# yao24/MPAS-Model

Hardware: AMD Instinct MI355X
Metric: dycore cell-updates/sec (nCells×nVertLevels/step) at 1/2/4/8 MI355X; % HBM roofline (higher is better)
Workload: dtype f64; 1 GPU; x1.163842 dry dycore, 56 levels, dt=360s (BASELINE.json configs[2] mesh; one full atm_srk3 per step); nCells=163842, nVertLevels=56, num_scalars=1, split_steps=3, acoustic_substeps=2, parallelism=single block, owned_cells_rank0=163842, halo_cells_rank0=0, hip_graph=True

## Files before the change

### mpas-model_amd/csrc/dycore.hip

```cpp
#include <hip/hip_runtime.h>
#include <rccl/rccl.h>

#include <algorithm>
#include <cmath>
#include <cstdio>
#include <cstring>
#include <functional>
#include <map>
#include <set>
#include <string>
#include <tuple>
#include <vector>
#include <unistd.h>

#ifdef MPAS_API_TAG
#include "api_rename.h"
#endif
#include "../../include/mpas_dycore.h"
#include "p2p_wire.h"
#include "kernels.hip"
#include "halo.hip"
#include "summary.hip"
#include "lbc.hip"
#include "model_init.hip"
// ... 67 lines not shown
  XSeg* d_pre = nullptr;
  XSeg* d_post = nullptr;
  int npre = 0, npost = 0, maxn_pre = 0, maxn_post = 0;
  double* sendbuf = nullptr;
  double* recvbuf = nullptr;
  std::vector<XMsg> rsend, rrecv;
  bool warmed = false;
  bool fused_pack = false;
  std::vector<PackMap> pack;
  bool fused_unpack = false;
  std::vector<UnpackMap> unpack;
  int fused_rec = 0;
  std::vector<XPack> rpk_cell, rpk_edge;
  std::vector<XUnpack> rup_cell, rup_edge;
  bool p2p = false;
  int p2p_id = -1;
  unsigned long long* p2p_cnt = nullptr;
  P2PGet* d_get = nullptr;
  int nget = 0, get_chunks = 0;
  unsigned long long** d_ready = nullptr;
  int nready = 0;
  const unsigned long long** d_cons = nullptr;
  int ncons = 0;
  bool pull = false;
  std::vector<XSeg> h_pre, h_post;
  std::vector<const std::vector<int32_t>*> h_pre_idx;
  std::vector<int64_t> h_pre_off, h_post_off;
  XSeg* d_local = nullptr;
  int nlocal = 0, maxn_local = 0;
  P2PSeg* d_pseg = nullptr;
  int2* d_chunk = nullptr;
  int nchunk = 0, npeer_work = 0;
  P2PPeer* d_peer = nullptr;
  bool skip_pull = false;
};

struct XField {
  const char* pool;
  const char* name;
  int tl;
  unsigned layers;
};
constexpr unsigned ALL_LAYERS = 0x7u;

}

struct mpas_dyc_ctx {
  Config cf{};
  int index_qv = 0;
  int device = 0;
  bool host_only = false;
  hipStream_t stream = nullptr;
  std::vector<Block> blk;
  int cur = 0;
  std::string err;
  hipEvent_t ev[8] = {};
  bool use_graph = false;
  bool graph_ran = false;
  std::map<std::string, hipGraphExec_t> graphs;
  std::map<std::string, double> graph_dt;
  int rank = 0, nranks = 1;
  ncclComm_t comm = nullptr;
  bool rccl_local = false;
  int loopback = 0;
  int p2p = 0;
  unsigned long long* p2p_flags = nullptr;
  int* p2p_status = nullptr;
  int* p2p_status_host = nullptr;
  std::vector<unsigned long long*> p2p_peer_flags;
  std::map<std::pair<int, uint64_t>, void*> p2p_fields;
  int p2p_nr = 0;
  int p2p_next = 0;
  std::vector<XField> p2p_open;
  bool p2p_pending = false;
  bool p2p_merge = true;
  bool p2p_pull = true;
  int p2p_release = 1;
  bool u_local = true;
  int halo_trim = 3;
  bool late_issue = false;
  bool overlap_all = false;
  bool fuse_tend_acoustic = true;
  bool fold_substep_avg = true;
  bool fold_rk1_edges = true;
  bool fuse_recover_diag = true;
  std::vector<XField> late_fs;
  bool late_pending = false;
  bool fused_pack_enabled = true;
  bool plain_exchange = false;
  bool lbc = false;
  bool planning = false;
  std::set<std::string> planned;
  std::map<std::string, XPlan> plans;
  std::vector<std::string>* record = nullptr;
  hipStream_t xstream = nullptr;
  hipEvent_t xfork = nullptr, xjoin = nullptr;
  int overlap = -1;
  bool bnd_ready = false;
  int physics = 0;
  int summary_flags = MPAS_DYC_PRINT_GLOBAL_MINMAX_VEL;
  int summary_tl = 0;
  IauState iau;
  ConvDiagState convdiag;
  MicropState microp;
  int64_t graph_captures = 0;
  bool tail_pending = false;
  bool profile = false;
  bool in_async = false;
  std::vector<hipEvent_t> prof_exposed, prof_rccl;
  hipEvent_t prof_step[2] = {};
  double prof_out[5] = {};
  char last_key[256] = {0};
  double* sum_gather = nullptr;
  mpas_dyc_allgather_fn host_allgather = nullptr;
  void* host_user = nullptr;
};

namespace {

#define HIPCHK(x)                                                                     \
  do {                                                                                \
    hipError_t e_ = (x);                                                              \
    if (e_ != hipSuccess) {                                                           \
      ctx->err = std::string(#x) + ": " + hipGetErrorString(e_);                      \
      return MPAS_DYC_EHIP;                                                           \
    }                                                                                 \
  } while (0)

#define NCCLCHK(x)                                                                    \
  do {                                                                                \
    ncclResult_t r_ = (x);                                                            \
    if (r_ != ncclSuccess) {                                                          \
      ctx->err = std::string(#x) + ": " + ncclGetErrorString(r_);                     \
      return MPAS_DYC_ECOMM;                                                          \
    }                                                                                 \
  } while (0)

#define CHK(x)                 \
  do {                         \
    int r__ = (x);             \
    if (r__) return r__;       \
  } while (0)

int64_t nloc(const Block& b, Loc l) {
  switch (l) {
    case L_CELL: return b.d.nCells + 1;
    case L_EDGE: return b.d.nEdges + 1;
    case L_VERTEX: return b.d.nVertices + 1;
    default: return 1;
  }
}

int64_t field_elems(const Block& b, const Field& f) { return nloc(b, f.loc) * f.inner; }
int64_t field_bytes(const Block& b, const Field& f) { return field_elems(b, f) * (f.is_int ? 4 : 8); }

bool is_host_0d(const Field& f) {
  return f.pool == "mesh" && (f.name == "cf1" || f.name == "cf2" || f.name == "cf3");
}

Field& add(Block& c, const char* pool, const char* name, Loc loc, int64_t inner, int ntl = 1, bool is_int = false,
           Target t = T_NONE) {
  Field f;
  f.pool = pool;
  f.name = name;
  f.loc = loc;
  f.inner = inner;
// ... 505 lines not shown
void swap_theta(mpas_dyc_ctx* ctx) {
  for (auto& b : ctx->blk) {
    Field* f = find(b, "state", "theta_m");
    std::swap(f->buf[0], f->buf[1]);
    f->flip ^= 1;
  }
}

Ptrs stage_pre(const Ptrs& p0, bool first_substep) {
  Ptrs p = p0;
  p.ru = p.ru_save;
  p.rw = p.rw_save;
  p.rw_rd = p.rw_save;
  p.rtheta_p = p.rtheta_p_save;
  p.theta_m2 = p.theta_m1;
  p.ru_rd = p.ru_save;
  p.theta_m2_rd = p.theta_m1;
  if (first_substep) {
    p.u2 = p.u1;
    p.w2 = p.w1;
    p.w2_rd = p.w1;
    p.rho_zz2 = p.rho_zz1;
    p.rho_zz2_rd = p.rho_zz1;
  }
  return p;
}

Ptrs stage_fin(const Ptrs& p0, bool first_substep) {
  Ptrs p = p0;
  p.rw_rd = p.rw_save;
  p.ru_rd = p.ru_save;
  p.theta_m2_rd = p.theta_m1;
  if (first_substep) {
    p.w2_rd = p.w1;
    p.rho_zz2_rd = p.rho_zz1;
  }
  return p;
}

int step_rotations(const Config& cf) { return cf.split_dynamics_transport ? cf.dynamics_split_steps : 1; }

void apply_step_rotations(mpas_dyc_ctx* ctx) {
  const int n = step_rotations(ctx->cf);
  if (n & 1) rotate_saves(ctx);
  if ((n - 1) & 1) swap_theta(ctx);
}

std::string layout_sig(mpas_dyc_ctx* ctx) {
  Block& b = ctx->blk[0];
  return std::to_string(ctx->cur) + "." + std::to_string(find(b, "diag", "ru")->rot_pos) + "." +
         std::to_string(find(b, "state", "theta_m")->flip);
}

struct Layout {
  std::vector<std::tuple<Field*, void*, void*, int, int>> f;
};
Layout save_layout(mpas_dyc_ctx* ctx) {
  Layout l;
  for (auto& b : ctx->blk)
    for (auto& f : b.fields)
      if (f.rot >= 0 || (f.pool == "state" && f.name == "theta_m")) l.f.emplace_back(&f, f.buf[0], f.buf[1], f.rot_pos, f.flip);
  return l;
}
void restore_layout(const Layout& l) {
  for (const auto& t : l.f) {
    Field* f = std::get<0>(t);
    f->buf[0] = std::get<1>(t);
    f->buf[1] = std::get<2>(t);
    f->rot_pos = std::get<3>(t);
    f->flip = std::get<4>(t);
  }
}

void rk_integration_setup(mpas_dyc_ctx* ctx, const Dims& d, const Ptrs& p) {
  CopyList c{};
  c.src[0] = p.scalars1;
  c.dst[0] = p.scalars2;
  c.n[0] = (int64_t)(d.nCells + 1) * d.K * d.ns;
  const unsigned gx = (unsigned)std::min<int64_t>((c.n[0] + 255) / 256, 2048);
  if (!ctx->planning) hipLaunchKernelGGL(k_copy_many, dim3(gx, 1), dim3(256), 0, ctx->stream, c);
}


void vert_imp_coefs(mpas_dyc_ctx* ctx, const Dims& d, const Ptrs& p, double dts) {
  if (g_vic == 2) {
    LAUNCH(k_vert_imp_coefs<true>, std::max(d.nCellsSolve, 1), d, p, dts, ctx->cf.epssm);
    if (d.nCellsSolve > 0 && !ctx->planning)
      hipLaunchKernelGGL(k_vert_imp_lu, dim3((unsigned)((d.nCellsSolve + 63) / 64)), dim3(64), 0, ctx->stream, d, p);
  } else if (pair_layout(d) && g_vic == 1) {
    LAUNCH_PE((k_vert_imp_coefs_p<false>), (k_vert_imp_coefs_p<true>), std::max(d.nCellsSolve, 1), d, p, dts, ctx->cf.epssm);
  } else {
    LAUNCH(k_vert_imp_coefs<false>, std::max(d.nCellsSolve, 1), d, p, dts, ctx->cf.epssm);
  }
}

bool fused_recover(const Dims& d) { return batched(d) && (d.maxEdges == 6 || d.maxEdges == 7); }

struct TendAcoustic {
  Ptrs pf;
  bool fin;
  double dts, rdt, invNs;
  int keep_pp, dl, store_tend;
  int sa;
  double sa_inv;
};
bool tend_acoustic_fused(const mpas_dyc_ctx* ctx, int rk_step, int nsub) {
#ifdef MPAS_WIDE
  return false;
#else
  if (!ctx->fuse_tend_acoustic || needs_exchange(ctx) || ctx->lbc || ctx->blk.size() != 1) return false;
  const Dims& d = ctx->blk[0].d;
  return fuse_smlstep(d) && fused_recover(d) && !(rk_step == 1 && nsub > 1);
#endif
}
bool substep_avg_folded(const mpas_dyc_ctx* ctx) {
#ifdef MPAS_WIDE
  return false;
#else
  if (!ctx->fold_substep_avg || needs_exchange(ctx) || ctx->lbc || ctx->blk.size() != 1) return false;
  if (!ctx->cf.split_dynamics_transport) return false;
  const Dims& d = ctx->blk[0].d;
  return pair_layout(d) && fused_recover(d) && d.nCellsSolve == d.nCells && d.nEdgesSolve == d.nEdges &&
         d.n_bnd_edges == 0;
#endif
}
bool rk1_edge_folded(const mpas_dyc_ctx* ctx, const Dims& d) {
#ifdef MPAS_WIDE
  return false;
#else
  return ctx->fold_rk1_edges && pair_layout(d) && !(ctx->cf.v_mom_eddy_visc2 > 0.0);
#endif
}
bool recover_diag_fused(const mpas_dyc_ctx* ctx) {
#ifdef MPAS_WIDE
  return false;
#else
  if (!ctx->fuse_recover_diag || needs_exchange(ctx) || ctx->lbc || ctx->blk.size() != 1) return false;
  if (ctx->cf.scalar_advection && !ctx->cf.split_dynamics_transport) return false;
  return pair_layout(ctx->blk[0].d);
#endif
}
void stage_sub_steps(const Config& cf, int n[3]) {
  const int nss = cf.number_of_sub_steps;
  n[0] = cf.time_integration_order == 3 ? 1 : std::max(1, nss / 2);
  n[1] = std::max(1, nss / 2);
  n[2] = nss;
}

void dyn_tend(mpas_dyc_ctx* ctx, const Dims& d, const Ptrs& p, int rk_step, double dt, int part = 0,
              bool hdiv_done = false, bool last = true, XPack tp = XPack{}, const TendAcoustic* ta = nullptr) {
  const Config& cf = ctx->cf;
  DynTendScal s{};
  s.rk_step = rk_step;
  s.store_phys_diag = last ? 1 : 0;
  s.dt = dt;
  s.invDt = 1.0 / dt;
  s.coef_3rd_order = cf.coef_3rd_order;
  s.c_s = cf.smagorinsky_coef;
  if (cf.horiz_mixing_smag) {
    s.h_mom_eddy_visc4 = cf.visc4_2dsmag * (cf.len_disp * cf.len_disp * cf.len_disp);
    s.h_theta_eddy_visc4 = s.h_mom_eddy_visc4;
  } else {
    s.h_mom_eddy_visc4 = cf.h_mom_eddy_visc4;
    s.h_theta_eddy_visc4 = cf.h_theta_eddy_visc4;
  }
  if (cf.rayleigh_damp_u)
    s.rayleigh_coef_inverse = 1.0 / ((double)cf.number_rayleigh_damp_u_levels *
                                     (cf.rayleigh_damp_u_timescale_days * SECONDS_PER_DAY));
  const bool bt = batched(d), m6 = d.maxEdges == 6;
  if (part != 2 && !(hdiv_done && rk_step > 1)) {
    if (!bt) LAUNCH(k_dyn_cells1, d.nCells, d, p, cf, s);
    else if (pair_layout(d) && g_cells1_pair && m6)
      LAUNCH_PE((k_dyn_cells1_p<6, false>), (k_dyn_cells1_p<6, true>), d.nCells, d, p, cf, s);
    else if (pair_layout(d) && g_cells1_pair)
      LAUNCH_PE((k_dyn_cells1_p<7, false>), (k_dyn_cells1_p<7, true>), d.nCells, d, p, cf, s);
    else if (m6) LAUNCH(k_dyn_cells1_b<6>, d.nCells, d, p, cf, s);
    else LAUNCH(k_dyn_cells1_b<7>, d.nCells, d, p, cf, s);
  }
  if (part == 1) return;
  auto delsq_vc = [&]() {
    if (!(s.h_mom_eddy_visc4 > 0.0)) return;
    if (pair_layout(d) && g_delsq_pair) {
      const int64_t nw = 3 * std::max<int64_t>((d.nVertices + 2 * PAIR_EPW - 1) / (2 * PAIR_EPW),
                                               (d.nCells + PAIR_EPW - 1) / PAIR_EPW);
      if (m6) LAUNCH_PE((k_dyn_delsq_vc_p<6, false>), (k_dyn_delsq_vc_p<6, true>), nw * PAIR_EPW, d, p);
      else LAUNCH_PE((k_dyn_delsq_vc_p<7, false>), (k_dyn_delsq_vc_p<7, true>), nw * PAIR_EPW, d, p);
    } else {
      const int nvc = 3 * std::max((d.nVertices + 1) / 2, d.nCells);
      if (m6) LAUNCH(k_dyn_delsq_vc_b<6>, nvc, d, p);
      else LAUNCH(k_dyn_delsq_vc_b<7>, nvc, d, p);
    }
  };
  const bool fold1 = rk_step == 1 && rk1_edge_folded(ctx, d);
  if (pair_layout(d)) {
    const int64_t nw = d.nEdges;
    if (rk_step == 1) LAUNCH_PE((k_dyn_edges_pgf_p<false>), (k_dyn_edges_pgf_p<true>), nw, d, p);
#ifndef MPAS_WIDE
    if (fold1) {
      delsq_vc();
      if (m6) LAUNCH_PE((k_dyn_edges_p<true, 10, true, false, true>), (k_dyn_edges_p<true, 10, true, true, true>), nw, d, p, cf, s, 1, tp);
      else LAUNCH_PE((k_dyn_edges_p<true, 12, true, false, true>), (k_dyn_edges_p<true, 12, true, true, true>), nw, d, p, cf, s, 1, tp);
    }
#endif
    if (d.maxEdges == 6 && rk_step == 1 && !fold1) LAUNCH_PE((k_dyn_edges_p<true, 10, true, false>), (k_dyn_edges_p<true, 10, true, true>), nw, d, p, cf, s, 0);
    if (d.maxEdges == 6 && rk_step != 1) LAUNCH_PE((k_dyn_edges_p<false, 10, false, false>), (k_dyn_edges_p<false, 10, false, true>), nw, d, p, cf, s, 1, tp);
    if (d.maxEdges == 7 && rk_step == 1 && !fold1) LAUNCH_PE((k_dyn_edges_p<true, 12, true, false>), (k_dyn_edges_p<true, 12, true, true>), nw, d, p, cf, s, 0);
    if (d.maxEdges == 7 && rk_step != 1) LAUNCH_PE((k_dyn_edges_p<false, 12, false, false>), (k_dyn_edges_p<false, 12, false, true>), nw, d, p, cf, s, 1, tp);
  } else if (batched(d)) {
    if (d.maxEdges == 6 && rk_step == 1) LAUNCH_E((k_dyn_edges_b<true, 10>), d.nEdges, d, p, cf, s, 0);
    if (d.maxEdges == 6 && rk_step != 1) LAUNCH_E((k_dyn_edges_b<false, 10>), d.nEdges, d, p, cf, s, 1);
    if (d.maxEdges == 7 && rk_step == 1) LAUNCH_E((k_dyn_edges_b<true, 12>), d.nEdges, d, p, cf, s, 0);
    if (d.maxEdges == 7 && rk_step != 1) LAUNCH_E((k_dyn_edges_b<false, 12>), d.nEdges, d, p, cf, s, 1);
  } else if (rk_step == 1)
    LAUNCH(k_dyn_edges<true>, d.nEdges, d, p, cf, s, 0);
  else
    LAUNCH(k_dyn_edges<false>, d.nEdges, d, p, cf, s, 1);
  if (rk_step == 1) {
    if (!bt) {
      if (s.h_mom_eddy_visc4 > 0.0) LAUNCH(k_dyn_delsq_vc, d.nVertices + d.nCells, d, p);
      LAUNCH(k_dyn_edges_rk1b, d.nEdgesSolve, d, p, cf, s);
      LAUNCH(k_dyn_cells2, d.nCells, d, p);
    } else {
      if (!fold1) {
        delsq_vc();
        LAUNCH(k_dyn_edges_rk1b_b, d.nEdgesSolve, d, p, cf, s, tp);
      }
      if (pair_layout(d) && g_cells2_pair) {
        if (m6) LAUNCH_PE((k_dyn_cells2_p<6, false>), (k_dyn_cells2_p<6, true>), d.nCells, d, p);
        else LAUNCH_PE((k_dyn_cells2_p<7, false>), (k_dyn_cells2_p<7, true>), d.nCells, d, p);
      } else if (m6) {
        LAUNCH(k_dyn_cells2_b<6>, d.nCells, d, p);
      } else {
        LAUNCH(k_dyn_cells2_b<7>, d.nCells, d, p);
      }
    }
  }
  if (!batched(d)) LAUNCH(k_dyn_advflux, d.nEdges, d, p);
  else if (pair_layout(d) && d.maxEdges == 6) LAUNCH_PE((k_dyn_advflux_p<10, false>), (k_dyn_advflux_p<10, true>), d.nEdges, d, p);
  else if (pair_layout(d)) LAUNCH_PE((k_dyn_advflux_p<12, false>), (k_dyn_advflux_p<12, true>), d.nEdges, d, p);
  else if (d.maxEdges == 6) LAUNCH_E(k_dyn_advflux_b<10>, d.nEdges, d, p);
  else LAUNCH_E(k_dyn_advflux_b<12>, d.nEdges, d, p);
#ifndef MPAS_WIDE
  if (ta) {
    const TendAcArgs a{ta->dts, cf.epssm, ta->rdt, ta->invNs, rk_step, ta->keep_pp, ta->dl,
                       ta->store_tend, ta->sa, ta->sa_inv};
    const bool m6 = d.maxEdges == 6, fin = ta->fin;
    if (m6 && rk_step == 1) LAUNCH((k_dyn_cells3_acoustic_r<6, true, true>), d.nCells, d, ta->pf, cf, s, a);
    if (m6 && rk_step != 1 && fin) LAUNCH((k_dyn_cells3_acoustic_r<6, false, true>), d.nCells, d, ta->pf, cf, s, a);
    if (m6 && rk_step != 1 && !fin) LAUNCH((k_dyn_cells3_acoustic_r<6, false, false>), d.nCells, d, ta->pf, cf, s, a);
    if (!m6 && rk_step == 1) LAUNCH((k_dyn_cells3_acoustic_r<7, true, true>), d.nCells, d, ta->pf, cf, s, a);
    if (!m6 && rk_step != 1 && fin) LAUNCH((k_dyn_cells3_acoustic_r<7, false, true>), d.nCells, d, ta->pf, cf, s, a);
    if (!m6 && rk_step != 1 && !fin) LAUNCH((k_dyn_cells3_acoustic_r<7, false, false>), d.nCells, d, ta->pf, cf, s, a);
    return;
  }
#endif
  if (batched(d)) {
    const bool sml = fuse_smlstep(d);
    if (d.maxEdges == 6 && rk_step == 1 && sml) LAUNCH((k_dyn_cells3_r<6, true, true>), d.nCellsSolve, d, p, cf, s);
    if (d.maxEdges == 6 && rk_step != 1 && sml) LAUNCH((k_dyn_cells3_r<6, false, true>), d.nCellsSolve, d, p, cf, s);
    if (d.maxEdges == 7 && rk_step == 1 && sml) LAUNCH((k_dyn_cells3_r<7, true, true>), d.nCellsSolve, d, p, cf, s);
    if (d.maxEdges == 7 && rk_step != 1 && sml) LAUNCH((k_dyn_cells3_r<7, false, true>), d.nCellsSolve, d, p, cf, s);
    if (d.maxEdges == 6 && rk_step == 1 && !sml) LAUNCH((k_dyn_cells3_r<6, true>), d.nCellsSolve, d, p, cf, s);
    if (d.maxEdges == 6 && rk_step != 1 && !sml) LAUNCH((k_dyn_cells3_r<6, false>), d.nCellsSolve, d, p, cf, s);
    if (d.maxEdges == 7 && rk_step == 1 && !sml) LAUNCH((k_dyn_cells3_r<7, true>), d.nCellsSolve, d, p, cf, s);
    if (d.maxEdges == 7 && rk_step != 1 && !sml) LAUNCH((k_dyn_cells3_r<7, false>), d.nCellsSolve, d, p, cf, s);
    return;
  }
  LAUNCH(k_dyn_cells3, d.nCellsSolve, d, p, cf, s);
}

void smlstep_pert(mpas_dyc_ctx* ctx, const Dims& d, const Ptrs& p, int phase, XUnpack tu_up = XUnpack{}) {
  if (fuse_smlstep(d)) {
    if (phase == 1) return;
    phase = 2;
  }
  const int64_t nb = phase == 2 ? d.n_bnd_cells : d.nCellsSolve;
  if (!batched(d)) LAUNCH(k_smlstep_pert, d.nCellsSolve, d, p, phase);
  else if (d.maxEdges == 6) LAUNCH(k_smlstep_pert_b<6>, nb, d, p, phase, tu_up);
  else LAUNCH(k_smlstep_pert_b<7>, nb, d, p, phase, tu_up);
}

void recover_cells3(mpas_dyc_ctx* ctx, const Dims& d, const Ptrs& p, int phase, int hdiv = 0) {
  if (!batched(d)) LAUNCH(k_recover_cells3, d.nCells, d, p, phase);
  else if (d.maxEdges == 6) LAUNCH(k_recover_cells3_b<6>, d.nCells, d, p, phase, hdiv);
  else LAUNCH(k_recover_cells3_b<7>, d.nCells, d, p, phase, hdiv);
}

double coef_divdamp(const mpas_dyc_ctx* ctx, double dts) {
  const double rdts = 1.0 / dts;
  return 2.0 * ctx->cf.smdiv * ctx->cf.len_disp * rdts;
}

void acoustic_edges(mpas_dyc_ctx* ctx, const Dims& d, const Ptrs& p, double dts, int small_step, int damp,
                    int phase, int fresh = 0, UnpackMap um = UnpackMap{}) {
  if (pair_layout(d)) {
    const int64_t nw = phase == 2 ? d.n_bnd_pairs : d.nEdges;
    const bool up = um.recv != nullptr;
    if (damp && up)
      LAUNCH_PE((k_acoustic_edges_p<true, true, false>), (k_acoustic_edges_p<true, true, true>), nw, d, p, dts, small_step, coef_divdamp(ctx, dts), phase, fresh, um);
    else if (damp)
      LAUNCH_PE((k_acoustic_edges_p<true, false, false>), (k_acoustic_edges_p<true, false, true>), nw, d, p, dts, small_step, coef_divdamp(ctx, dts), phase, fresh, um);
    else if (up)
      LAUNCH_PE((k_acoustic_edges_p<false, true, false>), (k_acoustic_edges_p<false, true, true>), nw, d, p, dts, small_step, 0.0, phase, fresh, um);
    else
      LAUNCH_PE((k_acoustic_edges_p<false, false, false>), (k_acoustic_edges_p<false, false, true>), nw, d, p, dts, small_step, 0.0, phase, fresh, um);
    return;
  }
  if (damp)
    LAUNCH_E(k_acoustic_edges<true>, d.nEdges, d, p, dts, small_step, coef_divdamp(ctx, dts), phase, fresh);
  else
    LAUNCH_E(k_acoustic_edges<false>, d.nEdges, d, p, dts, small_step, 0.0, phase, fresh);
}

void acoustic_cells(mpas_dyc_ctx* ctx, const Dims& d, const Ptrs& p, double dts, int small_step, int fin = 0,
                    double rdt = 0.0, double invNs = 0.0, int rk_step = 0, int keep_pp = 1, PackMap pk = PackMap{},
                    int dl = 0, XPack rp = XPack{}, int sa = 0, double sa_inv = 0.0) {
  if (batched(d) && d.maxEdges == 6) {
    if (fin)
      LAUNCH((k_acoustic_cells_r<6, true>), d.nCells, d, p, dts, small_step, ctx->cf.epssm, rdt, invNs, rk_step, keep_pp,
             pk, dl, rp, sa, sa_inv);
    else LAUNCH((k_acoustic_cells_r<6, false>), d.nCells, d, p, dts, small_step, ctx->cf.epssm, 0.0, 0.0, 0, 1, pk);
    return;
  }
  if (batched(d) && d.maxEdges == 7) {
    if (fin)
      LAUNCH((k_acoustic_cells_r<7, true>), d.nCells, d, p, dts, small_step, ctx->cf.epssm, rdt, invNs, rk_step, keep_pp,
             pk, dl, rp, sa, sa_inv);
    else LAUNCH((k_acoustic_cells_r<7, false>), d.nCells, d, p, dts, small_step, ctx->cf.epssm, 0.0, 0.0, 0, 1, pk);
    return;
  }
  LAUNCH(k_acoustic_cells, d.nCells, d, p, dts, small_step, ctx->cf.epssm);
}

inline int damping_delta(const mpas_dyc_ctx* ctx, const Dims& d, bool last_stage) {
  return (!needs_exchange(ctx) && !last_stage && pair_layout(d) && fused_recover(d)) ? 1 : 0;
}

bool fused_recover_edges(const Dims& d) { return pair_layout(d) && fused_recover(d); }

void divergence_damping(mpas_dyc_ctx* ctx, const Dims& d, const Ptrs& p, double dts, int phase, int fresh = 0,
                        double invNs = 0.0, UnpackMap um = UnpackMap{}, int dl = 0, XPack rp = XPack{},
                        XPack upk = XPack{}, int sa = 0, double sa_inv = 0.0) {
  const bool up = um.recv != nullptr;
  const int64_t nw = phase == 2 ? d.n_bnd_pairs : d.nEdges;
  const double cd = coef_divdamp(ctx, dts);
  if (pair_layout(d) && invNs > 0.0 && fused_recover_edges(d)) {
    if (up) LAUNCH_PE((k_divdamp_p<true, true, false>), (k_divdamp_p<true, true, true>), nw, d, p, cd, phase, dts, fresh, invNs, um, dl, rp, upk, sa, sa_inv);
    else LAUNCH_PE((k_divdamp_p<true, false, false>), (k_divdamp_p<true, false, true>), nw, d, p, cd, phase, dts, fresh, invNs, um, dl, rp, upk, sa, sa_inv);
  } else if (pair_layout(d)) {
    if (up) LAUNCH_PE((k_divdamp_p<false, true, false>), (k_divdamp_p<false, true, true>), nw, d, p, cd, phase, dts, fresh, 0.0, um, dl, rp);
    else LAUNCH_PE((k_divdamp_p<false, false, false>), (k_divdamp_p<false, false, true>), nw, d, p, cd, phase, dts, fresh, 0.0, um, dl, rp);
  }
  else LAUNCH(k_divdamp<DIVDAMP_EPW>, (d.nEdges + DIVDAMP_EPW - 1) / DIVDAMP_EPW, d, p, coef_divdamp(ctx, dts), phase,
              dts, fresh);
}

void solve_diagnostics(mpas_dyc_ctx* ctx, const Dims& d, const Ptrs& p, double dt, int tl, int rk_step ,
                       int store_grad = 1, XUnpack uu_up = XUnpack{}, int rec3_hdiv = -1) {
  const double* u = (tl == 1) ? p.u1 : p.u2;
  const double* h = (tl == 1) ? p.rho_zz1 : p.rho_zz2;
  const int reconstruct_v = (rk_step == 0 || rk_step == 3) ? 1 : 0;
  const int store_dv = (rk_step == 0 || rk_step == 3) ? 1 : 0;
  if (!batched(d)) {
    LAUNCH(k_diag_vertices, d.nVertices, d, p, u, store_dv);
    LAUNCH(k_diag_cells, d.nCells, d, p, u, ctx->cf.apvm_upwinding, store_dv);
    LAUNCH(k_diag_edges, d.nEdges, d, p, u, h, reconstruct_v, ctx->cf.apvm_upwinding, dt, store_grad);
    return;
  }
  if (pair_layout(d)) {
    LAUNCH_PE((k_diag_vertices_p<false>), (k_diag_vertices_p<true>), d.nVertices, d, p, u, store_dv, uu_up,
              (tl == 1) ? p.u1 : p.u2);
#ifndef MPAS_WIDE
    if (rec3_hdiv >= 0) {
      if (d.maxEdges == 6) LAUNCH(k_recover3_diag_cells_b<6>, d.nCells, d, p, rec3_hdiv, u, ctx->cf.apvm_upwinding, store_dv);
      else LAUNCH(k_recover3_diag_cells_b<7>, d.nCells, d, p, rec3_hdiv, u, ctx->cf.apvm_upwinding, store_dv);
    } else
#endif
    if (d.maxEdges == 6) LAUNCH(k_diag_cells_b<6>, d.nCells, d, p, u, ctx->cf.apvm_upwinding, store_dv);
    else LAUNCH(k_diag_cells_b<7>, d.nCells, d, p, u, ctx->cf.apvm_upwinding, store_dv);
    const int64_t nw = d.nEdges;
    if (d.maxEdges == 6) LAUNCH_PE((k_diag_edges_p<10, false>), (k_diag_edges_p<10, true>), nw, d, p, u, h, reconstruct_v, ctx->cf.apvm_upwinding, dt, store_grad);
    else LAUNCH_PE((k_diag_edges_p<12, false>), (k_diag_edges_p<12, true>), nw, d, p, u, h, reconstruct_v, ctx->cf.apvm_upwinding, dt, store_grad);
  } else if (d.maxEdges == 6) {
    LAUNCH(k_diag_vertices, d.nVertices, d, p, u, store_dv);
    LAUNCH(k_diag_cells_b<6>, d.nCells, d, p, u, ctx->cf.apvm_upwinding, store_dv);
    LAUNCH_E(k_diag_edges_b<10>, d.nEdges, d, p, u, h, reconstruct_v, ctx->cf.apvm_upwinding, dt, store_grad);
  } else {
    LAUNCH(k_diag_vertices, d.nVertices, d, p, u, store_dv);
    LAUNCH(k_diag_cells_b<7>, d.nCells, d, p, u, ctx->cf.apvm_upwinding, store_dv);
    LAUNCH_E(k_diag_edges_b<12>, d.nEdges, d, p, u, h, reconstruct_v, ctx->cf.apvm_upwinding, dt, store_grad);
  }
}

void advance_scalars(mpas_dyc_ctx* ctx, const Dims& d, const Ptrs& p, double dt, int rk_step, bool advance_density) {
  double wt_new = 1.0;
  if (advance_density) {
    if (rk_step == 1 && ctx->cf.time_integration_order == 3) wt_new = 1. / 3;
    if (rk_step == 1 && ctx->cf.time_integration_order == 2) wt_new = 1. / 2;
    if (rk_step == 2) wt_new = 1. / 2;
// ... 191 lines not shown
int lbc_scalars(mpas_dyc_ctx* ctx, const std::vector<Ptrs>& P, double dt, double dt_rk) {
  CHK(exchange(ctx, {{"state", "scalars", 2, ALL_LAYERS}}));
  EACH(LAUNCH(k_lbc_scalars_tmp, d.nCellsSolve, d, p, dt, dt_rk, dt_rk));
  EACH(LAUNCH(k_lbc_scalars_copy, d.nCellsSolve, d, p));
  return MPAS_DYC_OK;
}

#include "physics_host.hip"

int step_tail(mpas_dyc_ctx* ctx, const std::vector<Ptrs>& P, double dt) {
  if (ctx->lbc) {
    EACH(LAUNCH(k_lbc_reset_spec, d.nCellsSolve, d, p, dt));
    CHK(exchange(ctx, {{"state", "scalars", 2, ALL_LAYERS}}));
    EACH(LAUNCH(k_lbc_set_scalars, d.nCellsSolve, d, p, dt));
  }
  return summary_launch(ctx, 2);
}

int srk3(mpas_dyc_ctx* ctx, double dt) {
  const Config& cf = ctx->cf;
  std::vector<Ptrs> P = block_ptrs(ctx), Ppre, Pfin;
  auto relayout = [&](bool first_substep) {
    P = block_ptrs(ctx);
    Ppre.clear();
    Pfin.clear();
    for (const Ptrs& q : P) {
      Ppre.push_back(stage_pre(q, first_substep));
      Pfin.push_back(stage_fin(q, first_substep));
    }
  };
  int dynamics_split = cf.dynamics_split_steps;
  double dt_dynamics;
  if (cf.split_dynamics_transport) {
    dt_dynamics = dt / (double)dynamics_split;
  } else {
    dynamics_split = 1;
    dt_dynamics = dt;
  }
  const int nss = cf.number_of_sub_steps;
  double rk_timestep[3], rk_sub_timestep[3];
  int number_sub_steps[3];
  if (cf.time_integration_order == 3) {
    rk_timestep[0] = dt_dynamics / 3.;
    rk_timestep[1] = dt_dynamics / 2.;
    rk_timestep[2] = dt_dynamics;
    rk_sub_timestep[0] = dt_dynamics / 3.;
    rk_sub_timestep[1] = dt_dynamics / (double)nss;
    rk_sub_timestep[2] = dt_dynamics / (double)nss;
  } else {
    rk_timestep[0] = dt_dynamics / 2.;
    rk_timestep[1] = dt_dynamics / 2.;
    rk_timestep[2] = dt_dynamics;
    rk_sub_timestep[0] = dt_dynamics / (double)nss;
    rk_sub_timestep[1] = dt_dynamics / (double)nss;
    rk_sub_timestep[2] = dt_dynamics / (double)nss;
  }
  stage_sub_steps(cf, number_sub_steps);
  const bool scalars_in_dynamics = cf.scalar_advection && !cf.split_dynamics_transport;
  const bool split = split_phase(ctx);
  const bool lbc = ctx->lbc;
  CHK(exchange(ctx, {{"state", "theta_m", 1, ALL_LAYERS}, {"state", "scalars", 1, ALL_LAYERS},
                     {"diag", "pressure_p", 0, ALL_LAYERS}, {"diag", "rtheta_p", 0, ALL_LAYERS},
                     {"diag", "exner", 0, ALL_LAYERS}}));
  rotate_saves(ctx);
  relayout(true);
  EACH(rk_integration_setup(ctx, d, p));
  EACH(LAUNCH(k_moist_cells, d.nCells, d, p));
  EACH(if (pair_layout(d)) LAUNCH_PE((k_moist_edges_p<false>), (k_moist_edges_p<true>), d.nEdges, d, p);
       else LAUNCH(k_moist_edges, d.nEdges, d, p));
  if (iau_active(ctx)) CHK(iau_add_tend(ctx, P));

  auto xchg = [&](const std::vector<XField>& fs) { return split ? exchange_async(ctx, fs) : (exchange)(ctx, fs); };
  auto xwait = [&]() { return split ? exchange_wait(ctx) : MPAS_DYC_OK; };
  bool pending = false;
  bool final_pending = false;
  bool hdiv_prev = false;
  bool sml_fused = true, rec_overlap = false;
  for (const auto& b : ctx->blk) {
    sml_fused = sml_fused && fuse_smlstep(b.d);
    rec_overlap = rec_overlap || !fused_recover(b.d) || !fused_recover_edges(b.d);
  }
  if (ctx->overlap_all) sml_fused = false, rec_overlap = true;
  const bool avg_folded = substep_avg_folded(ctx);
  const bool rd_fused = recover_diag_fused(ctx);
  EACHV(Ppre, vert_imp_coefs(ctx, d, p, rk_sub_timestep[0]));
  for (int dynamics_substep = 1; dynamics_substep <= dynamics_split; ++dynamics_substep) {
    for (int rk_step = 1; rk_step <= 3; ++rk_step) {
      if (cf.time_integration_order == 3 && rk_step == 2) EACH(vert_imp_coefs(ctx, d, p, rk_sub_timestep[1]));
      const bool last_stage = dynamics_substep == dynamics_split && rk_step == 3;
      const bool hdiv_next = !lbc && rk_step < 3 && (!split || (rk_step == 1 && cf.time_integration_order == 3));
      const std::vector<Ptrs>& PS = rk_step == 1 ? Ppre : P;
      const std::vector<Ptrs>& PF = rk_step == 1 ? Pfin : P;
      const std::vector<XField> xtu = {{"tend", "u", 0, 0x1u}};
      const XPlan* xt = fused_rec_plan(ctx, xtu);
      auto tpk = [&](size_t ib) { return xt ? xt->rpk_edge[ib] : XPack{}; };
      auto tup = [&](size_t ib) { return xt ? xt->rup_edge[ib] : XUnpack{}; };
      const double dts = rk_sub_timestep[rk_step - 1];
      const int nsub = number_sub_steps[rk_step - 1];
      const bool fuse_ta = tend_acoustic_fused(ctx, rk_step, nsub);
      const int sa = (avg_folded && rk_step == 3)
                         ? SA_ON | (dynamics_substep == 1 ? SA_FIRST : 0) | (dynamics_substep == dynamics_split ? SA_LAST : 0)
                         : 0;
      const double sa_inv = 1.0 / (double)dynamics_split;
      TendAcoustic ta{};
      if (fuse_ta)
        ta = TendAcoustic{PF[0], nsub == 1, dts, rk_timestep[rk_step - 1], 1 / (double)nsub, last_stage ? 1 : 0,
                          nsub == 1 ? damping_delta(ctx, ctx->blk[0].d, last_stage) : 0, (nsub > 1 || last_stage) ? 1 : 0,
                          nsub == 1 ? sa : 0, sa_inv};
      const TendAcoustic* tap = fuse_ta ? &ta : nullptr;
      if (pending) {
        EACHV(PS, dyn_tend(ctx, d, p, rk_step, dt, 1, hdiv_prev && batched(d)));
        CHK(xwait());
        pending = false;
        EACHV(PS, dyn_tend(ctx, d, p, rk_step, dt, 2, false, last_stage, tpk(ib_), tap));
      } else {
        EACHV(PS, dyn_tend(ctx, d, p, rk_step, dt, 0, hdiv_prev && batched(d), last_stage, tpk(ib_), tap));
      }
      if (split && !sml_fused) {
        CHK(exchange_async(ctx, xtu));
        EACHV(PS, smlstep_pert(ctx, d, p, 1));
        CHK(exchange_wait(ctx));
        EACHV(PS, smlstep_pert(ctx, d, p, 2, tup(ib_)));
      } else if (split) {
        CHK(exchange(ctx, xtu));
        EACHV(PS, smlstep_pert(ctx, d, p, 2, tup(ib_)));
      } else {
        CHK(exchange(ctx, xtu));
        EACHV(PS, smlstep_pert(ctx, d, p, 0, tup(ib_)));
      }
      if (lbc) {
        const double tds = dt_dynamics * (double)(dynamics_substep - 1) + rk_timestep[rk_step - 1];
        EACHV(PS, LAUNCH(k_lbc_spec_tend_cells, d.nCellsSolve, d, p));
        EACHV(PS, LAUNCH(k_lbc_spec_tend_edges, d.nEdgesSolve, d, p));
        EACHV(PS, LAUNCH(k_lbc_relax_cells, d.nCellsSolve, d, p, dt, tds));
        EACHV(PS, LAUNCH(k_lbc_relax_edges, d.nEdges, d, p, dt, tds));
      }
      const unsigned rwp_layers = (!lbc && (ctx->halo_trim & 1)) ? 0x1u : ALL_LAYERS;
      const std::vector<XField> xrec = {{"diag", "rw_p", 0, rwp_layers}, {"diag", "ru_p", 0, ALL_LAYERS},
                                        {"diag", "rho_pp", 0, ALL_LAYERS}, {"diag", "rtheta_pp", 0, 0x2u}};
      const XPlan* xr = fused_rec_plan(ctx, xrec);
      auto rpc = [&](size_t ib) { return xr ? xr->rpk_cell[ib] : XPack{}; };
      auto rpe = [&](size_t ib) { return xr ? xr->rpk_edge[ib] : XPack{}; };
      auto ruc = [&](size_t ib) { return xr ? xr->rup_cell[ib] : XUnpack{}; };
      auto rue = [&](size_t ib) { return xr ? xr->rup_edge[ib] : XUnpack{}; };
      const std::vector<XField> xu = {{"state", "u", 2, ALL_LAYERS}};
      const bool u_skip = ctx->u_local && !lbc && rk_step < 3;
      const XPlan* xuu = u_skip ? nullptr : fused_rec_plan(ctx, xu);
      auto upk = [&](size_t ib) { return xuu ? xuu->rpk_edge[ib] : XPack{}; };
      auto uup = [&](size_t ib) { return xuu ? xuu->rup_edge[ib] : XUnpack{}; };
      const XPlan* unpack_xp = nullptr;
      auto um_of = [&](size_t ib) { return unpack_xp ? unpack_xp->unpack[ib] : UnpackMap{}; };
      for (int small_step = 1; small_step <= nsub; ++small_step) {
        if (small_step == 1) {
        } else if (split) {
          EACHV(PS, acoustic_edges(ctx, d, p, dts, small_step, 1, 1, small_step == 2));
          CHK(exchange_wait(ctx));
          EACHV(PS, acoustic_edges(ctx, d, p, dts, small_step, 1, 2, small_step == 2, um_of(ib_)));
        } else {
          EACHV(PS, acoustic_edges(ctx, d, p, dts, small_step, 1, 0, small_step == 2, um_of(ib_)));
        }
        unpack_xp = nullptr;
        std::vector<XField> xf = {{"diag", "rtheta_pp", 0, 0x1u}};
        if (small_step < nsub) xf.push_back({"diag", "rho_pp", 0, 0x1u});
        const XPlan* xp = fused_pack_plan(ctx, xf);
        if (!(fuse_ta && small_step == 1))
          EACHV(small_step == nsub ? PF : PS,
              acoustic_cells(ctx, d, p, dts, small_step, small_step == nsub, rk_timestep[rk_step - 1],
                            1 / (double)nsub, rk_step, needs_exchange(ctx) || last_stage,
                            xp ? xp->pack[ib_] : PackMap{}, damping_delta(ctx, d, last_stage),
                            small_step == nsub ? rpc(ib_) : XPack{}, small_step == nsub ? sa : 0, sa_inv));
        if (split) {
          CHK(exchange_async(ctx, xf));
        } else {
          CHK((exchange)(ctx, xf));
        }
        if (xp && xp->fused_unpack) unpack_xp = xp;
      }
      if (split) {
        EACH(divergence_damping(ctx, d, p, dts, 1, nsub == 1, 1 / (double)nsub, UnpackMap{}, 0, rpe(ib_), upk(ib_)));
        CHK(exchange_wait(ctx));
        EACH(divergence_damping(ctx, d, p, dts, 2, nsub == 1, 0.0, um_of(ib_), 0, rpe(ib_)));
      } else {
        EACH(divergence_damping(ctx, d, p, dts, 0, nsub == 1, 1 / (double)nsub, um_of(ib_),
                                damping_delta(ctx, d, last_stage), rpe(ib_), upk(ib_), sa, sa_inv));
      }
      const double invNs = 1 / (double)number_sub_steps[rk_step - 1];
      const double rdt = rk_timestep[rk_step - 1];
      if (split) {
        if (rec_overlap) CHK(exchange_async(ctx, xrec));
        else CHK((exchange)(ctx, xrec));
        EACH(if (!fused_recover(d)) LAUNCH(k_recover_cells1, d.nCells + 1, d, p, rdt, invNs, rk_step, 1, 0));
        EACH(if (!fused_recover_edges(d)) LAUNCH(k_recover_edges, d.nEdges, d, p, invNs, 1, XUnpack{}, upk(ib_)));
        if (rec_overlap) CHK(exchange_wait(ctx));
        EACH(LAUNCH(k_recover_cells1, d.nCells + 1 - d.nCellsSolve, d, p, rdt, invNs, rk_step, 2, d.nCellsSolve,
                    ruc(ib_)));
        EACH(LAUNCH(k_recover_edges, d.n_bnd_edges, d, p, invNs, 2, rue(ib_), upk(ib_)));
        if (lbc) {
          EACH(recover_cells3(ctx, d, p, 0));
          EACH(LAUNCH(k_lbc_u, d.nEdges, d, p, dt_dynamics * (double)(dynamics_substep - 1) + rk_timestep[rk_step - 1]));
          CHK(exchange(ctx, {{"state", "u", 2, ALL_LAYERS}}));
        } else if (u_skip) {
          EACH(recover_cells3(ctx, d, p, 0, hdiv_next));
        } else {
          CHK(exchange_async(ctx, {{"state", "u", 2, ALL_LAYERS}}));
          EACH(recover_cells3(ctx, d, p, 0, hdiv_next));
          CHK(exchange_wait(ctx));
        }
      } else {
        CHK((exchange)(ctx, xrec));
        EACH(if (fused_recover(d)) LAUNCH(k_recover_cells1, d.nCells + 1 - d.nCellsSolve, d, p, rdt, invNs, rk_step, 2,
                                          d.nCellsSolve, ruc(ib_));
             else LAUNCH(k_recover_cells1, d.nCells + 1, d, p, rdt, invNs, rk_step, 0, 0, ruc(ib_)));
        EACH(if (!fused_recover_edges(d)) LAUNCH(k_recover_edges, d.nEdges, d, p, invNs, 0, rue(ib_), upk(ib_));
             else LAUNCH(k_recover_edges, d.n_bnd_edges, d, p, invNs, 2, rue(ib_), upk(ib_)));
        if (!rd_fused) EACH(recover_cells3(ctx, d, p, 0, hdiv_next));
        if (lbc)
          EACH(LAUNCH(k_lbc_u, d.nEdges, d, p, dt_dynamics * (double)(dynamics_substep - 1) + rk_timestep[rk_step - 1]));
        if (!u_skip) CHK(exchange(ctx, {{"state", "u", 2, ALL_LAYERS}}));
      }
      if (scalars_in_dynamics) {
        if (rk_step < 3 || (!cf.monotonic && !cf.positive_definite)) {
          EACH(advance_scalars(ctx, d, p, rk_timestep[rk_step - 1], rk_step, false));
        } else {
          CHK(advance_scalars_mono(ctx, P, rk_timestep[rk_step - 1], false));
        }
        if (lbc) CHK(lbc_scalars(ctx, P, dt, rk_timestep[rk_step - 1]));
      }
      EACH(solve_diagnostics(ctx, d, p, dt, 2, rk_step,
                             dynamics_substep == dynamics_split && rk_step == 3, uup(ib_),
                             rd_fused ? (hdiv_next ? 1 : 0) : -1));
      const unsigned pve_layers = (!lbc && (ctx->halo_trim & 2)) ? 0x3u : ALL_LAYERS;
      std::vector<XField> xd = {{"state", "w", 2, ALL_LAYERS}, {"diag", "pv_edge", 0, pve_layers},
                                {"diag", "rho_edge", 0, pve_layers}};
      if (scalars_in_dynamics) xd.push_back({"state", "scalars", 2, ALL_LAYERS});
      if (lbc) {
        CHK((exchange)(ctx, xd));
        EACH(LAUNCH(k_lbc_zero_grad_w, d.nCellsSolve, d, p));
        CHK((exchange)(ctx, {{"state", "w", 2, ALL_LAYERS}}));
        if (rk_step == 3 && dynamics_substep < dynamics_split) {
          CHK((exchange)(ctx, {{"state", "theta_m", 2, ALL_LAYERS}, {"diag", "pressure_p", 0, ALL_LAYERS},
                               {"diag", "rtheta_p", 0, ALL_LAYERS}, {"diag", "exner", 0, ALL_LAYERS}}));
          EACH(vert_imp_coefs(ctx, d, p, rk_sub_timestep[0]));
        }
      } else if (rk_step < 3) {
        CHK(xchg(xd));
        pending = true;
      } else if (dynamics_substep < dynamics_split) {
        xd.insert(xd.end(), {{"state", "theta_m", 2, ALL_LAYERS}, {"diag", "pressure_p", 0, ALL_LAYERS},
                             {"diag", "rtheta_p", 0, ALL_LAYERS}, {"diag", "exner", 0, ALL_LAYERS}});
        CHK(xchg(xd));
        EACH(vert_imp_coefs(ctx, d, p, rk_sub_timestep[0]));
        CHK(xwait());
      } else if (split) {
        CHK(exchange_async(ctx, xd));
        final_pending = true;
      } else {
        CHK((exchange)(ctx, xd));
      }
      hdiv_prev = hdiv_next;
    }
    if (!ctx->planning && !avg_folded)
      EACH(hipLaunchKernelGGL(k_substep_finish_v, dim3(2048), dim3(BLOCK_THREADS), 0, ctx->stream, d, p,
                              dynamics_substep, dynamics_split, 1.0 / (double)dynamics_split));
    if (dynamics_substep < dynamics_split) {
      rotate_saves(ctx);
      swap_theta(ctx);
      relayout(false);
    }
    if (final_pending) {
      CHK(exchange_wait(ctx));
      final_pending = false;
    }
  }

  if (cf.scalar_advection && cf.split_dynamics_transport) {
    double rk_ts[3] = {dt / 3., dt / 2., dt};
    if (cf.time_integration_order == 2) rk_ts[0] = dt / 2.;
    const bool mono3 = cf.monotonic || cf.positive_definite;
    for (int rk_step = 1; rk_step <= 3; ++rk_step) {
      if (rk_step < 3 || !mono3) {
        EACH(advance_scalars(ctx, d, p, rk_ts[rk_step - 1], rk_step, true));
      } else {
        CHK(advance_scalars_mono(ctx, P, rk_ts[rk_step - 1], true, true));
      }
      if (lbc) CHK(lbc_scalars(ctx, P, dt, rk_ts[rk_step - 1]));
      if (rk_step == 2 && mono3) {
        mono_prep(ctx, P, rk_ts[2], true);
        CHK(exchange(ctx, {{"state", "scalars", 2, ALL_LAYERS}, {"state", "scalars", 1, ALL_LAYERS}}));
      } else if (rk_step < 3) {
        CHK(exchange(ctx, {{"state", "scalars", 2, ALL_LAYERS}}));
      }
    }
  }
  EACH(reconstruct(ctx, d, p, p.u2));
  if (physics_tendencies(ctx)) {
    if (ctx->physics & MPAS_DYC_PHYSICS_RQVDYNTEN)
      EACH(LAUNCH(k_physics_rqvdynten, d.nCells + 1, d, p, ctx->index_qv, cf.monotonic, dt));
    for (auto& b : ctx->blk) {
      const int64_t n = (int64_t)b.d.ns * (b.d.nCells + 1) * b.d.K;
      if (!ctx->planning)
        hipLaunchKernelGGL(k_physics_clip_scalars, dim3((unsigned)std::min<int64_t>((n + 255) / 256, 4096)),
                           dim3(256), 0, ctx->stream, ::P<double>(ctx, b, "state", "scalars", 2), n);
    }
    if (ctx->microp.scheme == MPAS_DYC_MICROP_KESSLER) CHK(kessler_enqueue(ctx, dt, 2));
  }
  if (!(ctx->physics & MPAS_DYC_PHYSICS_MICROPHYSICS)) CHK(step_tail(ctx, P, dt));
  return MPAS_DYC_OK;
}

int init_diagnostics(mpas_dyc_ctx* ctx, double dt, bool coupled = true) {
  const std::vector<Ptrs> P = block_ptrs(ctx);
  CHK(exchange(ctx, {{"state", "u", 1, ALL_LAYERS}}));
  if (coupled) {
    EACH(LAUNCH(k_init_coupled_a, d.nCells, d, p, ctx->index_qv));
    EACH(LAUNCH(k_init_coupled_b, d.nEdges, d, p));
    EACH(LAUNCH(k_init_coupled_c, d.nCells, d, p));
  }
  EACH(solve_diagnostics(ctx, d, p, dt, 1, 0));
  EACH(reconstruct(ctx, d, p, p.u1));
  CHK(exchange(ctx, {{"diag", "pv_edge", 0, ALL_LAYERS}, {"diag", "ru", 0, ALL_LAYERS},
                     {"diag", "rw", 0, ALL_LAYERS}}));
  return MPAS_DYC_OK;
}

}

namespace {

int fill_dims(Dims& d, const mpas_dyc_dims* dims) {
#ifdef MPAS_WIDE
  constexpr int lo = WIDE_THREADS == 128 ? MPAS_DYC_MAX_LEVELS_WAVE : MPAS_DYC_MAX_LEVELS_WIDE;
  if (dims->nVertLevels <= lo || dims->nVertLevels >= WIDE_THREADS || dims->nVertLevels > MPAS_DYC_MAX_LEVELS)
    return MPAS_DYC_EINVAL;
  static_assert(WIDE_THREADS % 64 == 0 && WIDE_THREADS >= 128 && WIDE_THREADS <= 512,
// ... 171 lines not shown

int mpas_dyc_create_blocks(int32_t nblocks, const mpas_dyc_dims* dims, const mpas_dyc_config* cfg, int device,
                           mpas_dyc_ctx** out) {
  if (!dims || !cfg || !out || nblocks < 1) return MPAS_DYC_EINVAL;
  *out = nullptr;
  mpas_dyc_ctx* ctx = new mpas_dyc_ctx();
  ctx->blk.resize(nblocks);
  for (int b = 0; b < nblocks; ++b) {
    if (fill_dims(ctx->blk[b].d, &dims[b]) != MPAS_DYC_OK || dims[b].nVertLevels != dims[0].nVertLevels ||
        dims[b].num_scalars != dims[0].num_scalars) {
      delete ctx;
      return MPAS_DYC_EINVAL;
    }
    ctx->blk[b].me_decl = dims[b].maxEdges;
    ctx->blk[b].me2_decl = dims[b].maxEdges2;
  }
  ctx->index_qv = dims[0].index_qv - 1;
  fill_config(ctx->cf, cfg);
  if (ctx->cf.time_integration_order != 2 && ctx->cf.time_integration_order != 3) {
    delete ctx;
    return MPAS_DYC_EINVAL;
  }
  if (const char* ul = getenv("MPAS_DYCORE_U_LOCAL")) ctx->u_local = std::string(ul) != "0";
  if (const char* ht = getenv("MPAS_DYCORE_HALO_TRIM")) ctx->halo_trim = std::atoi(ht);
  if (device == MPAS_DYC_HOST_ONLY) {
    ctx->host_only = true;
    for (auto& b : ctx->blk) build_registry(b);
    *out = ctx;
    return MPAS_DYC_OK;
  }
  if (device >= 0 && hipSetDevice(device) != hipSuccess) {
    delete ctx;
    return MPAS_DYC_EHIP;
  }
  (void)hipGetDevice(&ctx->device);
  if (hipStreamCreateWithFlags(&ctx->stream, hipStreamNonBlocking) != hipSuccess) {
    delete ctx;
    return MPAS_DYC_EHIP;
  }
  for (auto& e : ctx->ev) (void)hipEventCreate(&e);
  if (hipStreamCreateWithFlags(&ctx->xstream, hipStreamNonBlocking) != hipSuccess ||
      hipEventCreateWithFlags(&ctx->xfork, hipEventDisableTiming) != hipSuccess ||
      hipEventCreateWithFlags(&ctx->xjoin, hipEventDisableTiming) != hipSuccess) {
    mpas_dyc_destroy(ctx);
    return MPAS_DYC_EHIP;
  }
  if (const char* kt = getenv("MPAS_DYCORE_KERNELS")) {
    const std::string t(kt);
    g_kernel_tier = t == "general" ? 0 : t == "batched" ? 1 : 2;
  } else {
    g_kernel_tier = 2;
  }
  g_fuse_smlstep = 1;
  if (const char* fs = getenv("MPAS_DYCORE_FUSE_SMLSTEP")) g_fuse_smlstep = std::string(fs) != "0";
  g_mono_pairs = 1;
  if (const char* mp = getenv("MPAS_DYCORE_MONO_PAIRS")) g_mono_pairs = std::string(mp) != "0";
  g_delsq_pair = 1;
  if (const char* dp = getenv("MPAS_DYCORE_DELSQ_PAIR")) g_delsq_pair = std::string(dp) != "0";
  g_cells2_pair = 1;
  if (const char* cp = getenv("MPAS_DYCORE_CELLS2_PAIR")) g_cells2_pair = std::string(cp) != "0";
  g_cells1_pair = 1;
  if (const char* c1 = getenv("MPAS_DYCORE_CELLS1_PAIR")) g_cells1_pair = std::string(c1) != "0";
#if defined(MPAS_WIDE) && WIDE_THREADS > 128
  g_vic = 2;
#else
  g_vic = 1;
#endif
  if (const char* vm = getenv("MPAS_DYCORE_VIC")) {
    const std::string v(vm);
    g_vic = v == "column" ? 0 : v == "pair" ? 1 : v == "split" ? 2 : g_vic;
  }
  g_mono_fuse = MONO_FUSE_BOUNDS;
  if (const char* mf = getenv("MPAS_DYCORE_MONO_FUSE")) g_mono_fuse = std::atoi(mf);
  if (const char* fp = getenv("MPAS_DYCORE_FUSED_PACK")) ctx->fused_pack_enabled = std::string(fp) != "0";
  if (const char* lb = getenv("MPAS_DYCORE_LOOPBACK")) ctx->loopback = std::atoi(lb);
  if (const char* pp = getenv("MPAS_DYCORE_P2P")) ctx->p2p = std::atoi(pp);
  if (const char* pm = getenv("MPAS_DYCORE_P2P_MERGE")) ctx->p2p_merge = std::atoi(pm) != 0;
  if (const char* pu = getenv("MPAS_DYCORE_P2P_PULL")) ctx->p2p_pull = std::atoi(pu) != 0;
  if (const char* pr = getenv("MPAS_DYCORE_P2P_RELEASE")) ctx->p2p_release = std::atoi(pr) != 0;
  if (const char* li = getenv("MPAS_DYCORE_LATE_ISSUE")) ctx->late_issue = std::string(li) == "1";
  if (const char* oa = getenv("MPAS_DYCORE_OVERLAP_ALL")) ctx->overlap_all = std::string(oa) == "1";
  if (const char* ft = getenv("MPAS_DYCORE_FUSE_TEND_ACOUSTIC")) ctx->fuse_tend_acoustic = std::string(ft) != "0";
  if (const char* fs = getenv("MPAS_DYCORE_FOLD_SUBSTEP_AVG")) ctx->fold_substep_avg = std::string(fs) != "0";
  if (const char* fe = getenv("MPAS_DYCORE_FOLD_RK1_EDGES")) ctx->fold_rk1_edges = std::string(fe) != "0";
  if (const char* fr = getenv("MPAS_DYCORE_FUSE_RECOVER_DIAG")) ctx->fuse_recover_diag = std::string(fr) != "0";
  if (const char* ov = getenv("MPAS_DYCORE_OVERLAP")) ctx->overlap = std::atoi(ov);
  for (auto& b : ctx->blk) {
    build_registry(b);
    for (auto& f : b.fields) {
      if (f.group != G_ALWAYS) continue;
      const int64_t nb = field_bytes(b, f) + 256;
      for (int t = 0; t < f.ntl; ++t) {
        if (hipMalloc(&f.buf[t], nb) != hipSuccess || hipMemset(f.buf[t], 0, nb) != hipSuccess) {
          mpas_dyc_destroy(ctx);
          return MPAS_DYC_EHIP;
        }
      }
      if (is_host_0d(f)) f.buf[1] = new double(0.0);
    }
    const size_t nf = 2 + (size_t)b.d.ns;
    if (hipMalloc(&b.sum_part, (size_t)SUM_MAX_FIELDS * SUM_PARTS * SUM_REC * sizeof(double)) != hipSuccess ||
        hipMalloc(&b.sum_out, nf * SUM_REC * sizeof(double)) != hipSuccess) {
      mpas_dyc_destroy(ctx);
      return MPAS_DYC_EHIP;
    }
  }
  *out = ctx;
  return MPAS_DYC_OK;
}

int mpas_dyc_create(const mpas_dyc_dims* dims, const mpas_dyc_config* cfg, int device, mpas_dyc_ctx** out) {
  return mpas_dyc_create_blocks(1, dims, cfg, device, out);
}

void mpas_dyc_destroy(mpas_dyc_ctx* ctx) {
  if (!ctx) return;
  if (ctx->host_only) {
    delete ctx;
    return;
  }
  (void)hipSetDevice(ctx->device);
  if (ctx->stream) (void)hipStreamSynchronize(ctx->stream);
  if (getenv("MPAS_DYCORE_P2P_DEBUG"))
    for (const auto& kv : ctx->plans)
      if (kv.second.p2p_id >= 0 && kv.second.p2p_cnt) {
        unsigned long long c[2] = {0, 0};
        (void)hipMemcpy(c, kv.second.p2p_cnt, sizeof(c), hipMemcpyDeviceToHost);
        printf("p2pdbg rank %d id %d uses %llu wg %llu nget %d %s\n", ctx->rank, kv.second.p2p_id, c[0], c[1],
               kv.second.nget, kv.first.c_str());
      }
  invalidate_plans(ctx);
  for (auto& b : ctx->blk) {
    for (auto& f : b.fields) {
      for (int t = 0; t < f.ntl; ++t)
        if (f.buf[t]) (void)hipFree(f.buf[t]);
      if (f.packed) (void)hipFree(f.packed);
      if (is_host_0d(f)) delete (double*)f.buf[1];
    }
    for (auto& x : b.xl) {
      if (x.d_idx) (void)hipFree(x.d_idx);
      if (x.d_pos) (void)hipFree(x.d_pos);
    }
    if (b.sum_part) (void)hipFree(b.sum_part);
    if (b.sum_out) (void)hipFree(b.sum_out);
    if (b.cv.start) (void)hipFree(b.cv.start);
    if (b.cv.kite) (void)hipFree(b.cv.kite);
  }
  if (ctx->sum_gather) (void)hipFree(ctx->sum_gather);
  p2p_teardown(ctx);
  if (ctx->comm) ncclCommDestroy(ctx->comm);
  for (auto& e : ctx->ev)
    if (e) (void)hipEventDestroy(e);
  for (auto& e : ctx->prof_step)
    if (e) (void)hipEventDestroy(e);
  if (ctx->xfork) (void)hipEventDestroy(ctx->xfork);
  if (ctx->xjoin) (void)hipEventDestroy(ctx->xjoin);
  if (ctx->xstream) (void)hipStreamDestroy(ctx->xstream);
  if (ctx->stream) (void)hipStreamDestroy(ctx->stream);
  delete ctx;
}

const char* mpas_dyc_last_error(const mpas_dyc_ctx* ctx) { return ctx ? ctx->err.c_str() : "null context"; }

int32_t mpas_dyc_num_blocks(const mpas_dyc_ctx* ctx) { return ctx ? (int32_t)ctx->blk.size() : 0; }

int64_t mpas_dyc_block_field_bytes(const mpas_dyc_ctx* ctx, int32_t block, const char* pool, const char* name) {
  if (!ctx || !pool || !name || block < 0 || block >= (int32_t)ctx->blk.size()) return 0;
  const Block& b = ctx->blk[block];
  auto it = b.by_name.find(std::string(pool) + "." + name);
  if (it == b.by_name.end()) return 0;
  const Field& f = b.fields[it->second];
  if (GROUPS[f.group].hidden && !f.buf[0]) return 0;
  return field_bytes(b, f);
}

int64_t mpas_dyc_field_bytes(const mpas_dyc_ctx* ctx, const char* pool, const char* name) {
  return mpas_dyc_block_field_bytes(ctx, 0, pool, name);
}

void* mpas_dyc_block_field_device_ptr(mpas_dyc_ctx* ctx, int32_t block, const char* pool, const char* name,
                                      int32_t time_level) {
  Block* b = get_block(ctx, block);
  if (!b || !pool || !name) return nullptr;
  Field* f = find(*b, pool, name);
  if (!f) return nullptr;
  if (f->me || (f->pool == "mesh" && (f->name == "zb_cell" || f->name == "zb3_cell"))) ctx->bnd_ready = false;
  return f->buf[slot_of(ctx, *f, time_level)];
}

void* mpas_dyc_field_device_ptr(mpas_dyc_ctx* ctx, const char* pool, const char* name, int32_t time_level) {
  return mpas_dyc_block_field_device_ptr(ctx, 0, pool, name, time_level);
}

int mpas_dyc_set_block_field(mpas_dyc_ctx* ctx, int32_t block, const char* pool, const char* name,
                             int32_t time_level, const void* host, int64_t nbytes) {
  if (!ctx || !pool || !name || !host) return MPAS_DYC_EINVAL;
  CHK(require_device(ctx));
  Block* bp = get_block(ctx, block);
  if (!bp) {
    ctx->err = "no block " + std::to_string(block);
    return MPAS_DYC_EINVAL;
  }
  Block& b = *bp;
  Field* f = find(b, pool, name);
  if (!f) {
    ctx->err = std::string("unknown field ") + pool + "." + name;
    return MPAS_DYC_EINVAL;
  }
  if (is_host_0d(*f)) {
    if (nbytes != 8) return MPAS_DYC_EINVAL;
    *(double*)f->buf[1] = *(const double*)host;
    HIPCHK(hipMemcpy(f->buf[0], host, 8, hipMemcpyHostToDevice));
    return MPAS_DYC_OK;
  }
  const int64_t nb = field_bytes(b, *f);
  if (nbytes != nb) {
    ctx->err = "size mismatch for " + f->pool + "." + f->name + ": got " + std::to_string(nbytes) + " expected " +
               std::to_string(nb);
    return MPAS_DYC_EINVAL;
  }
  const int slot = slot_of(ctx, *f, time_level);
  HIPCHK(hipSetDevice(ctx->device));
  if (!f->buf[slot])
    CHK(f->group == G_ON_SET ? alloc_field(ctx, b, *f, false)
                             : alloc_group(ctx, f->group, GROUPS[f->group].all_blocks ? nullptr : &b));
  if (f->me) ctx->bnd_ready = false;
  if (f->is_int && f->target != T_NONE) {
    const int64_t n = field_elems(b, *f);
    std::vector<int32_t> tmp(n);
    const int32_t* src = (const int32_t*)host;
    const int64_t nt = target_n(b, f->target);
    for (int64_t i = 0; i < n; ++i) {
      int32_t v = src[i] - 1;
      if (f->target == T_SMALL) v = v < 0 ? 0 : v;
      else if (v < 0 || v > nt) v = (int32_t)nt;
      tmp[i] = v;
    }
    if (f->pool == "mesh" && f->name == "cellsOnEdge") {
      count_active_edges(b, src);
      b.h_coe = tmp;
      ctx->bnd_ready = false;
    }
    if (f->pool == "mesh" && f->name == "edgesOnCell") {
      b.h_eoc = tmp;
      ctx->bnd_ready = false;
    }
    if (f->pool == "mesh" && f->name == "cellsOnVertex") {
      b.h_cov = tmp;
      b.cv.ready = false;
      if (group_ready(ctx, G_CONVDIAG)) ctx->bnd_ready = false;
    }
    if (f->pool == "mesh" && (f->name == "verticesOnEdge" || f->name == "edgesOnVertex")) {
      (f->name == "verticesOnEdge" ? b.h_voe : b.h_eov) = tmp;
      if (!ctx->plans.empty()) invalidate_plans(ctx);
    }
    HIPCHK(hipMemcpyAsync(f->buf[slot], tmp.data(), nb, hipMemcpyHostToDevice, ctx->stream));
    HIPCHK(hipStreamSynchronize(ctx->stream));
  } else if (f->nsub > 1) {
    const int64_t n = nloc(b, f->loc), ns = f->nsub, m = f->inner / ns;
    const double* src = (const double*)host;
    std::vector<double> tmp(n * f->inner);
    for (int64_t c = 0; c < n; ++c)
      for (int64_t k = 0; k < m; ++k)
        for (int64_t s = 0; s < ns; ++s) tmp[(s * n + c) * m + k] = src[(c * m + k) * ns + s];
    HIPCHK(hipMemcpyAsync(f->buf[slot], tmp.data(), nb, hipMemcpyHostToDevice, ctx->stream));
    HIPCHK(hipStreamSynchronize(ctx->stream));
  } else {
    HIPCHK(hipMemcpyAsync(f->buf[slot], host, nb, hipMemcpyHostToDevice, ctx->stream));
    HIPCHK(hipStreamSynchronize(ctx->stream));
    if (f->pool == "mesh" && f->name == "nEdgesOnCell") {
      b.h_noc.assign((const int32_t*)host, (const int32_t*)host + nb / 4);
      ctx->bnd_ready = false;
    }
    if (f->pool == "mesh" && f->name == "nEdgesOnEdge") {
      b.h_noe.assign((const int32_t*)host, (const int32_t*)host + nb / 4);
      ctx->bnd_ready = false;
    }
    if (f->pool == "mesh" && (f->name == "zb_cell" || f->name == "zb3_cell")) ctx->bnd_ready = false;
    if (f->pool == "tend" && f->name == "rt_diabatic_tend") {
      const double* h = (const double*)host;
      int nz = 0;
      for (int64_t i = 0; i < nb / 8 && !nz; ++i) nz = h[i] != 0.0;
      b.d.diabatic = nz || ctx->microp.scheme;
    }
  }
  return MPAS_DYC_OK;
}

int mpas_dyc_set_field(mpas_dyc_ctx* ctx, const char* pool, const char* name, int32_t time_level,
                       const void* host, int64_t nbytes) {
  return mpas_dyc_set_block_field(ctx, 0, pool, name, time_level, host, nbytes);
}

int mpas_dyc_get_block_field(mpas_dyc_ctx* ctx, int32_t block, const char* pool, const char* name,
                             int32_t time_level, void* host, int64_t nbytes) {
  if (!ctx || !pool || !name || !host) return MPAS_DYC_EINVAL;
  CHK(require_device(ctx));
  Block* bp = get_block(ctx, block);
  if (!bp) {
    ctx->err = "no block " + std::to_string(block);
    return MPAS_DYC_EINVAL;
  }
  Block& b = *bp;
  Field* f = find(b, pool, name);
  if (!f) {
    ctx->err = std::string("unknown field ") + pool + "." + name;
    return MPAS_DYC_EINVAL;
  }
  if (is_host_0d(*f)) {
// ... 810 lines not shown
      *q++ = '\n';
    }
    *q = '\0';
  }
  return (nm > cap || kl > keys_bytes) ? MPAS_DYC_EINVAL : MPAS_DYC_OK;
}

int mpas_dyc_shift_time_levels(mpas_dyc_ctx* ctx) {
  if (!ctx) return MPAS_DYC_EINVAL;
  ctx->cur ^= 1;
  return MPAS_DYC_OK;
}

int mpas_dyc_synchronize(mpas_dyc_ctx* ctx) {
  if (!ctx) return MPAS_DYC_EINVAL;
  if (ctx->host_only) return MPAS_DYC_ESTATE;
  HIPCHK(hipSetDevice(ctx->device));
  HIPCHK(hipStreamSynchronize(ctx->stream));
  HIPCHK(hipStreamSynchronize(ctx->xstream));
  return p2p_check(ctx);
}

int mpas_dyc_set_p2p(mpas_dyc_ctx* ctx, int32_t on) {
  if (!ctx) return MPAS_DYC_EINVAL;
  if (on < 0) return MPAS_DYC_OK;
  invalidate_plans(ctx);
  ctx->p2p = on != 0;
  return MPAS_DYC_OK;
}

int mpas_dyc_get_p2p(const mpas_dyc_ctx* ctx) { return ctx && ctx->p2p ? 1 : 0; }

int mpas_dyc_set_overlap(mpas_dyc_ctx* ctx, int32_t on) {
  if (!ctx) return MPAS_DYC_EINVAL;
  invalidate_plans(ctx);
  ctx->overlap = on < 0 ? -1 : (on != 0);
  return MPAS_DYC_OK;
}

int mpas_dyc_use_graph(mpas_dyc_ctx* ctx, int32_t on) {
  if (!ctx) return MPAS_DYC_EINVAL;
  ctx->use_graph = on != 0;
  return MPAS_DYC_OK;
}

int mpas_dyc_block_layout(mpas_dyc_ctx* ctx, int32_t block, int32_t* out) {
  Block* b = get_block(ctx, block);
  if (!b || !out) return MPAS_DYC_EINVAL;
  if (ctx->host_only) return MPAS_DYC_ESTATE;
  HIPCHK(hipSetDevice(ctx->device));
  if (!ctx->bnd_ready) CHK(compute_bnd(ctx));
  out[0] = b->d.maxEdges;
  out[1] = b->d.maxEdges2;
  out[2] = pair_layout(b->d) ? 2 : batched(b->d) ? 1 : 0;
#ifdef MPAS_WIDE
  out[3] = WIDE_THREADS == 128 ? 1 : WIDE_THREADS == 256 ? 2 : WIDE_THREADS == 512 ? 3
           : WIDE_THREADS == 192 ? 4 : WIDE_THREADS == 320 ? 5 : WIDE_THREADS == 384 ? 6 : 7;
#else
  out[3] = 0;
#endif
  return MPAS_DYC_OK;
}

int mpas_dyc_fused_tend_acoustic(mpas_dyc_ctx* ctx) {
  if (!ctx || ctx->host_only) return 0;
  if (hipSetDevice(ctx->device) != hipSuccess) return 0;
  if (!ctx->bnd_ready && compute_bnd(ctx) != MPAS_DYC_OK) return 0;
  int nsub[3], m = 0;
  stage_sub_steps(ctx->cf, nsub);
  for (int rk = 1; rk <= 3; ++rk)
    if (tend_acoustic_fused(ctx, rk, nsub[rk - 1])) m |= 1 << (rk - 1);
  return m;
}

int mpas_dyc_folded_passes(mpas_dyc_ctx* ctx) {
  if (!ctx || ctx->host_only) return 0;
  if (hipSetDevice(ctx->device) != hipSuccess) return 0;
  if (!ctx->bnd_ready && compute_bnd(ctx) != MPAS_DYC_OK) return 0;
  int m = substep_avg_folded(ctx) ? 1 : 0;
  bool all = !ctx->blk.empty();
  for (const auto& b : ctx->blk) all = all && rk1_edge_folded(ctx, b.d);
  if (all) m |= 2;
  if (recover_diag_fused(ctx)) m |= 4;
  return m;
}

double mpas_dyc_acoustic_bytes(const mpas_dyc_ctx* ctx) {
  if (!ctx) return 0.0;
  const Dims& d = ctx->blk[0].d;
  const double K = d.K;
  const double nEact = ctx->blk[0].nEdges_act >= 0 ? (double)ctx->blk[0].nEdges_act : (double)d.nEdges;
  const double nC = d.nCellsSolve;
  return 8.0 * (K * (7.0 * nEact + 18.0 * nC) + 9.0 * (K + 1.0) * nC);
}

int mpas_dyc_time_acoustic_step(mpas_dyc_ctx* ctx, double dts, int32_t small_step, int32_t reps, double* ms_out,
                                double* ms_kernels) {
  if (!ctx || reps < 1) return MPAS_DYC_EINVAL;
  if (ctx->host_only) return MPAS_DYC_ESTATE;
  HIPCHK(hipSetDevice(ctx->device));
  if (!ctx->bnd_ready) CHK(compute_bnd(ctx));
  Block& b = ctx->blk[0];
  const Ptrs p = make_ptrs(ctx, b);
  const Dims& d = b.d;
  double acc[3] = {0, 0, 0};
  float t;
  std::vector<hipEvent_t> ev(2 * (size_t)reps + 2);
  for (auto& e : ev) HIPCHK(hipEventCreateWithFlags(&e, hipEventDisableSystemFence));
  auto destroy = [&]() {
    for (auto& e : ev) (void)hipEventDestroy(e);
  };
  HIPCHK(hipEventRecord(ev[0], ctx->stream));
  for (int r = 0; r < reps; ++r) {
    acoustic_edges(ctx, d, p, dts, small_step, r > 0 ? 1 : 0, 0);
    HIPCHK(hipEventRecord(ev[2 * r + 1], ctx->stream));
    acoustic_cells(ctx, d, p, dts, small_step);
    HIPCHK(hipEventRecord(ev[2 * r + 2], ctx->stream));
  }
  divergence_damping(ctx, d, p, dts, 0);
  const size_t e_end = 2 * (size_t)reps + 1;
  HIPCHK(hipEventRecord(ev[e_end], ctx->stream));
  HIPCHK(hipStreamSynchronize(ctx->stream));
  (void)hipEventElapsedTime(&t, ev[2 * (size_t)reps], ev[e_end]);
  acc[2] += t;
  for (int r = 0; ms_kernels && r < reps; ++r) {
    (void)hipEventElapsedTime(&t, ev[2 * r], ev[2 * r + 1]);
    acc[0] += t;
    (void)hipEventElapsedTime(&t, ev[2 * r + 1], ev[2 * r + 2]);
    acc[1] += t;
  }
  float tot;
  (void)hipEventElapsedTime(&tot, ev[0], ev[e_end]);
  destroy();
  if (ms_out) *ms_out = tot / reps;
  if (ms_kernels)
    for (int i = 0; i < 3; ++i) ms_kernels[i] = acc[i] / reps;
  return MPAS_DYC_OK;
}

}
```

### mpas-model_amd/csrc/kernels.hip

```cpp
#include "dycore.h"

namespace mpas {

#ifdef MPAS_WIDE
#ifndef WIDE_THREADS
#define WIDE_THREADS 128
#endif
#define WAVES_PER_BLOCK 1
#define BLOCK_THREADS WIDE_THREADS
#else
#ifndef WAVES_PER_BLOCK
#define WAVES_PER_BLOCK 4
#endif
#define BLOCK_THREADS (64 * WAVES_PER_BLOCK)
#endif

__device__ __forceinline__ int xcd_block() {
#ifdef NO_XCD_REMAP
  return blockIdx.x;
#endif
  const int nb = gridDim.x, bid = blockIdx.x;
  const int q = nb >> 3, r = nb & 7, x = bid & 7, i = bid >> 3;
  return x * q + min(x, r) + i;
}
// ... 253 lines not shown
    int e = d.nEdges, o = d.nCells;
    if (i < ne && i < d.maxEdges) {
      e = eoc[(size_t)c * d.maxEdges + i];
      if (e >= 0 && e < d.nEdges) {
        const int c1 = coe[2 * e], c2 = coe[2 * e + 1];
        o = (c1 == c) ? c2 : c1;
      } else {
        e = d.nEdges;
      }
    }
    rec[(size_t)c * CELL_REC + i] = e;
    rec[(size_t)c * CELL_REC + CELL_REC_ME + i] = o;
    if (i < d.maxEdges)
      cdv[(size_t)c * d.maxEdges + i] = (i < ne) ? sign[(size_t)c * d.maxEdges + i] * dvEdge[e] : 0.0;
  }
  int bits = 0;
  for (int i = 0; i < CELL_REC_ME && i < d.maxEdges; ++i) {
    if (i >= ne) continue;
    const double sg = sign[(size_t)c * d.maxEdges + i];
    bits |= (sg > 0.0 ? 0 : (sg < 0.0 ? 1 : 2)) << (2 * i);
    const int e = rec[(size_t)c * CELL_REC + i];
    if (e < d.nEdges && coe[2 * e] == c) bits |= 1 << (16 + i);
  }
  rec[(size_t)c * CELL_REC + 14] = ne;
  rec[(size_t)c * CELL_REC + 15] = bits;
}

template <int ME>
struct CellSten {
  int e[ME], o[ME];
  int ne, bits;
  __device__ __forceinline__ double sg(int i) const {
    const int s = (bits >> (2 * i)) & 3;
    return s == 0 ? 1.0 : (s == 1 ? -1.0 : 0.0);
  }
  __device__ __forceinline__ bool first(int i) const { return (bits >> (16 + i)) & 1; }
};
template <int ME>
__device__ __forceinline__ CellSten<ME> load_sten(const Ptrs& p, int c) {
  CellSten<ME> s;
  const int* r = p.cell_rec + (size_t)c * CELL_REC;
#pragma unroll
  for (int i = 0; i < ME; ++i) {
    s.e[i] = r[i];
    s.o[i] = r[CELL_REC_ME + i];
  }
  s.ne = r[14];
  s.bits = r[15];
  return s;
}

__device__ __forceinline__ int rec_off(const XUnpack& u, int f, int i, int nsolve) {
  return (u.recv && i >= nsolve && i - nsolve < u.nh) ? u.off[(size_t)f * u.nh + (i - nsolve)] : -1;
}

__global__ __launch_bounds__(BLOCK_THREADS) void k_moist_cells(Dims d, Ptrs p) {
  const int c = wave_elem(0);
  if (c >= d.nCells) return;
  const int k = lane_id(), K = d.K;
  const bool act = k < K;
  double q = 0.0;
  if (act) {
    for (int iq = d.moist_start; iq <= d.moist_end; ++iq) q = q + p.scalars2[SIX(c, k, iq)];
    p.qtot[(size_t)c * K + k] = q;
  }
  double qm = up1(q);
  if (act && k >= 1) {
    double qtotal = 0.5 * (q + qm);
    p.cqw[(size_t)c * K + k] = 1.0 / (1.0 + qtotal);
  }
}

__global__ __launch_bounds__(BLOCK_THREADS) void k_moist_edges(Dims d, Ptrs p) {
  const int e = wave_elem(0);
  if (e >= d.nEdges) return;
  const int c1 = p.cellsOnEdge[2 * e], c2 = p.cellsOnEdge[2 * e + 1];
  if (!(c1 < d.nCellsSolve || c2 < d.nCellsSolve)) return;
  const int k = lane_id(), K = d.K;
  if (k >= K) return;
  double qtotal = 0.0;
  for (int iq = d.moist_start; iq <= d.moist_end; ++iq)
    qtotal = qtotal + 0.5 * (p.scalars2[SIX(c1, k, iq)] + p.scalars2[SIX(c2, k, iq)]);
  p.cqu[(size_t)e * K + k] = 1.0 / (1.0 + qtotal);
}

template <bool SPLIT = false>
__global__ __launch_bounds__(BLOCK_THREADS) void k_vert_imp_coefs(Dims d, Ptrs p, double dts, double epssm) {
  const int c = wave_elem(0);
  const int k = lane_id(), K = d.K;
  const double dtseps = .5 * dts * (1. + epssm);
  const double rcv = RGAS / (CP - RGAS);
  const double c2 = CP * rcv;
  if (blockIdx.x == 0)
    for (int k = threadIdx.x; k < K; k += blockDim.x) p.cofrz[k] = dtseps * p.rdzw[k];
  if (c >= d.nCellsSolve) return;
  const bool act = k < K;
  const size_t o = (size_t)c * K + k;
  const double zz = LD(p.zz, o), pp = LD(p.exner, o), t = LD(p.theta_m2, o);
  const double rb = LD(p.rho_base, o), rtb = LD(p.rtheta_base, o), pb = LD(p.exner_base, o);
  const double rt = LD(p.rtheta_p, o), cqw = LD(p.cqw, o), qtot = LD(p.qtot, o);
  const double fzm = act ? p.fzm[k] : 0.0, fzp = act ? p.fzp[k] : 0.0;
  const double rdzu = act ? p.rdzu[k] : 0.0, rdzw = act ? p.rdzw[k] : 0.0;
  const double zzm = up1(zz), pm = up1(pp), tm = up1(t);
  double cofwr = 0.0, cofwz = 0.0, coftz = 0.0;
  if (act && k >= 1) {
    cofwr = .5 * dtseps * GRAVITY * (fzm * zz + fzp * zzm);
    cofwz = dtseps * c2 * (fzm * zz + fzp * zzm) * rdzu * cqw * (fzm * pp + fzp * pm);
    coftz = dtseps * (fzm * t + fzp * tm);
  }
  double cofwt = 0.0;
  if (act) cofwt = .5 * dtseps * rcv * zz * GRAVITY * rb / (1. + qtot) * pp / ((rtb + rt) * pb);
  const double coftz_p = dn1(coftz), coftz_m = up1(coftz);
  const double cofwt_m = up1(cofwt), rdzw_m = up1(rdzw);
  const double cofrz = dtseps * rdzw, cofrz_m = up1(cofrz);
  double a = 0.0, b = 1.0, cc = 0.0;
  if (act && k >= 1) {
    a = -cofwz * coftz_m * rdzw_m * zzm + cofwr * cofrz_m - cofwt_m * coftz_m * rdzw_m;
    b = 1. + cofwz * (coftz * rdzw * zz + coftz * rdzw_m * zzm) - coftz * (cofwt * rdzw - cofwt_m * rdzw_m) +
        cofwr * (cofrz - cofrz_m);
    cc = -cofwz * coftz_p * rdzw * zz - cofwr * cofrz + cofwt * coftz_p * rdzw;
  }
  double alpha = 0.0, gamma = 0.0;
#ifdef MPAS_WIDE
  if constexpr (SPLIT) {
    alpha = b;
    gamma = cc;
  } else {
    column_lu(a, b, cc, k, K, alpha, gamma);
  }
#else
  if constexpr (SPLIT) {
    alpha = b;
    gamma = cc;
  } else {
    for (int kk = 1; kk < K; ++kk) {
      const double gp = readlane_d(gamma, kk - 1);
      if (k == kk) {
        alpha = 1. / (b - a * gp);
        gamma = cc * alpha;
      }
    }
  }
#endif
  if (act) {
    if (k >= 1) {
      p.cofwr[o] = cofwr;
      p.cofwz[o] = cofwz;
    }
    p.cofwt[o] = cofwt;
    p.a_tri[o] = a;
    p.alpha_tri[o] = alpha;
    p.gamma_tri[o] = gamma;
  }
  if (k <= K) p.coftz[(size_t)c * (K + 1) + k] = coftz;
}

__global__ __launch_bounds__(64) void k_vert_imp_lu(Dims d, Ptrs p) {
  constexpr int LU_CHUNK = 16, SEGS = 64 / LU_CHUNK;
  __shared__ double sa[64][LU_CHUNK + 1], sb[64][LU_CHUNK + 1], sc[64][LU_CHUNK + 1];
  const int c0 = blockIdx.x * 64, lane = threadIdx.x;
  const int ncol = min(64, d.nCellsSolve - c0);
  const int K = d.K;
  const int seg = lane / LU_CHUNK, kk = lane % LU_CHUNK;
  if (lane < ncol) {
    p.alpha_tri[(size_t)(c0 + lane) * K] = 0.0;
    p.gamma_tri[(size_t)(c0 + lane) * K] = 0.0;
  }
  double g = 0.0;
  for (int k0 = 1; k0 < K; k0 += LU_CHUNK) {
    const int nk = min(LU_CHUNK, K - k0);
    double va[LU_CHUNK], vb[LU_CHUNK], vc[LU_CHUNK];
#pragma unroll
    for (int jj = 0; jj < LU_CHUNK; ++jj) {
      const int j = seg + SEGS * jj;
      if (j < ncol && kk < nk) {
        const size_t o = (size_t)(c0 + j) * K + k0 + kk;
        va[jj] = p.a_tri[o];
        vb[jj] = p.alpha_tri[o];
        vc[jj] = p.gamma_tri[o];
      }
    }
#pragma unroll
    for (int jj = 0; jj < LU_CHUNK; ++jj) {
      const int j = seg + SEGS * jj;
      if (j < ncol && kk < nk) {
        sa[j][kk] = va[jj];
        sb[j][kk] = vb[jj];
        sc[j][kk] = vc[jj];
      }
    }
    __syncthreads();
    if (lane < ncol) {
      double aa[LU_CHUNK], bb[LU_CHUNK], cc[LU_CHUNK];
#pragma unroll
      for (int j = 0; j < LU_CHUNK; ++j) {
        aa[j] = sa[lane][j];
        bb[j] = sb[lane][j];
        cc[j] = sc[lane][j];
      }
#pragma unroll
      for (int j = 0; j < LU_CHUNK; ++j)
        if (j < nk) {
          const double al = 1. / (bb[j] - aa[j] * g);
// ... 2027 lines not shown
  const int2 ceB = *reinterpret_cast<const int2*>(p.cellsOnEdge + 2 * eB);
  const int2 veA = *reinterpret_cast<const int2*>(p.verticesOnEdge + 2 * eA);
  const int2 veB = *reinterpret_cast<const int2*>(p.verticesOnEdge + 2 * eB);
  int neoe = 0;
  int eoe[NE2];
  double wgt[NE2];
  if (reconstruct_v) {
    neoe = sel(h, p.nEdgesOnEdge[eA], p.nEdgesOnEdge[eB]);
#pragma unroll
    for (int j = 0; j < NE2; ++j) {
      eoe[j] = sel(h, p.edgesOnEdge[(size_t)eA * d.maxEdges2 + j], p.edgesOnEdge[(size_t)eB * d.maxEdges2 + j]);
      wgt[j] = sel(h, ld_uniform_f64(p.weightsOnEdge + (size_t)eA * d.maxEdges2 + j),
                   ld_uniform_f64(p.weightsOnEdge + (size_t)eB * d.maxEdges2 + j));
    }
  }
  double invDv = 0.0, invDc = 0.0;
  d2 ue{};
  if (apvm > 0.0) {
    invDv = sel(h, ld_uniform_f64(p.invDvEdge + eA), ld_uniform_f64(p.invDvEdge + eB));
    invDc = sel(h, ld_uniform_f64(p.invDcEdge + eA), ld_uniform_f64(p.invDcEdge + eB));
    ue = ld2(u + o);
  }
  const int c1 = sel(h, ceA.x, ceB.x), c2 = sel(h, ceA.y, ceB.y), v1 = sel(h, veA.x, veB.x), v2 = sel(h, veA.y, veB.y);
  const d2 h1 = ld2(hh + (size_t)c1 * K + 2 * lc), h2 = ld2(hh + (size_t)c2 * K + 2 * lc);
  const d2 pv1 = ld2(p.pv_vertex + (size_t)v1 * K + 2 * lc), pv2 = ld2(p.pv_vertex + (size_t)v2 * K + 2 * lc);
  d2 pc1{}, pc2{};
  if (apvm > 0.0) {
    pc1 = ld2(p.pv_cell + (size_t)c1 * K + 2 * lc);
    pc2 = ld2(p.pv_cell + (size_t)c2 * K + 2 * lc);
  }
  const bool st = (h == 0 || hasB) && 2 * l < K;
  d2 vv;
  if (reconstruct_v) {
    d2 uu[NE2];
#pragma unroll
    for (int j = 0; j < NE2; ++j) uu[j] = ld2(u + (size_t)eoe[j] * K + 2 * lc);
    vv = d2{0.0, 0.0};
#pragma unroll
    for (int j = 0; j < NE2; ++j) {
      if (j < neoe) {
        vv.x = vv.x + wgt[j] * uu[j].x;
        vv.y = vv.y + wgt[j] * uu[j].y;
      }
    }
    if (st) pst(p.v + o, vv, two);
  } else {
    vv = ld2(p.v + o);
  }
  if (st) pst(p.rho_edge + o, d2{0.5 * (h1.x + h2.x), 0.5 * (h1.y + h2.y)}, two);
  d2 pve{0.5 * (pv1.x + pv2.x), 0.5 * (pv1.y + pv2.y)};
  if (apvm > 0.0) {
    const double r = apvm * dt;
    const double r1 = 1.0 * invDv;
    const double r2 = 1.0 * invDc;
    const d2 gt{(pv2.x - pv1.x) * r1, (pv2.y - pv1.y) * r1};
    const d2 gn{(pc2.x - pc1.x) * r2, (pc2.y - pc1.y) * r2};
    if (st && store_grad) {
      pst(p.gradPVt + o, gt, two);
      pst(p.gradPVn + o, gn, two);
    }
    pve.x = pve.x - r * (vv.x * gt.x + ue.x * gn.x);
    pve.y = pve.y - r * (vv.y * gt.y + ue.y * gn.y);
  }
  if (st) pst(p.pv_edge + o, pve, two);
}

template <bool ODD>
__device__ __forceinline__ d2 ld_pp(const Dims& d, const Ptrs& p, const UnpackMap& um, int which, int c, int lc,
                                    bool st) {
  double* fld = which ? p.rho_pp : p.rtheta_pp;
  const size_t o = (size_t)c * d.K + 2 * lc;
  const int* map = which ? um.rho : um.rt;
  if (map && c >= d.nCellsSolve && c < d.nCells) {
    const int off = map[c - d.nCellsSolve];
    if (off >= 0) {
      const d2 v = ld2(um.recv + off + 2 * lc);
      if (st) pst(fld + o, v, !ODD || 2 * lc + 1 < d.K);
      return v;
    }
  }
  return ld2(fld + o);
}

enum { SA_ON = 1, SA_FIRST = 2, SA_LAST = 4 };
__device__ __forceinline__ void store_avg(double* avg, double* split, size_t i, double a, int sa, double inv) {
  if (!sa) {
    avg[i] = a;
    return;
  }
  const double s = (sa & SA_FIRST) ? a : a + split[i];
  split[i] = s;
  if (sa & SA_LAST) avg[i] = s * inv;
}

template <bool REC = false, bool UP = false, bool ODD = false>
__global__ __launch_bounds__(PAIR_THREADS) void k_divdamp_p(Dims d, Ptrs p, double coef_divdamp, int phase, double dts,
                                                            int fresh, double invNs = 0.0, UnpackMap um = UnpackMap{},
                                                            int dl = 0, XPack rp = XPack{}, XPack upk = XPack{},
                                                            int sa = 0, double sa_inv = 0.0) {
  int eA, eB;
  bool hasB;
  if (!pair_edges(d, p, phase, eA, eB, hasB)) return;
  const int K = d.K, h = pair_half(), l = pair_lane();
  const int lc = min(l, (ODD ? K + 1 : K) / 2 - 1);
  const bool two = !ODD || 2 * l + 1 < K;
  const int e = sel(h, eA, eB);
  const size_t o = (size_t)e * K + 2 * lc;
  const int2 ceA = *reinterpret_cast<const int2*>(p.cellsOnEdge + 2 * eA);
  const int2 ceB = *reinterpret_cast<const int2*>(p.cellsOnEdge + 2 * eB);
  const int bA = phase ? p.edge_bnd[eA] : 0, bB = phase ? p.edge_bnd[eB] : 0;
  d2 ru;
  if (fresh) {
    const d2 tu = ld2(p.tend_u + o);
    ru = d2{dts * tu.x, dts * tu.y};
  } else {
    ru = ld2(p.ru_p + o);
  }
  const double mask = sel(h, ld_uniform_f64(p.specZoneMaskEdge + eA), ld_uniform_f64(p.specZoneMaskEdge + eB));
  auto active = [&](int2 ce, int bnd) {
    return (ce.x < d.nCellsSolve || ce.y < d.nCellsSolve) && (phase == 0 || ((bnd != 0) == (phase == 2)));
  };
  const bool onA = active(ceA, bA), onB = hasB && active(ceB, bB);
  if (!onA && !onB) return;
  const size_t o1 = (size_t)sel(h, ceA.x, ceB.x) * K + 2 * lc, o2 = (size_t)sel(h, ceA.y, ceB.y) * K + 2 * lc;
  const bool lv = 2 * l < K && (h ? onB : onA);
  d2 dd1, dd2;
  if (dl) {
    dd1 = ld2(p.rtheta_pp_old + o1);
    dd2 = ld2(p.rtheta_pp_old + o2);
  } else {
    const d2 r1 = UP ? ld_pp<ODD>(d, p, um, 0, sel(h, ceA.x, ceB.x), lc, lv) : ld2(p.rtheta_pp + o1);
    const d2 r2 = UP ? ld_pp<ODD>(d, p, um, 0, sel(h, ceA.y, ceB.y), lc, lv) : ld2(p.rtheta_pp + o2);
    const d2 q1 = ld2(p.rtheta_pp_old + o1), q2 = ld2(p.rtheta_pp_old + o2);
    dd1 = d2{r1.x - q1.x, r1.y - q1.y};
    dd2 = d2{r2.x - q2.x, r2.y - q2.y};
  }
  const d2 t1 = ld2(p.theta_m1 + o1), t2 = ld2(p.theta_m1 + o2);
  d2 out;
  out.x = ru.x + coef_divdamp * (-(dd2.x) - -(dd1.x)) * (1.0 - mask) / (t1.x + t2.x);
  out.y = ru.y + coef_divdamp * (-(dd2.y) - -(dd1.y)) * (1.0 - mask) / (t1.y + t2.y);
  pack_rec_edge(rp, d, eA, eB, hasB, h, lc, (h ? onB : onA) && 2 * l < K, two, out);
  if (!REC) {
    if ((h ? onB : onA) && 2 * l < K) {
      pst(p.ru_p + o, out, two);
      if (fresh) pst(p.ruAvg + o, ru, two);
    }
    return;
  }
  const bool rA = onA && (phase ? bA : p.edge_bnd[eA]) == 0;
  const bool rB = onB && (phase ? bB : p.edge_bnd[eB]) == 0;
  const d2 rs = ld2(p.ru_save + o);
  const d2 ra = fresh ? ru : ld2(p.ruAvg + o);
  const d2 sp = (sa && !(sa & SA_FIRST)) ? ld2(p.ruAvg_split + o) : d2{0.0, 0.0};
  const d2 z1 = ld2(p.rho_zz2 + o1), z2 = ld2(p.rho_zz2 + o2);
  const d2 rr{rs.x + out.x, rs.y + out.y};
  const d2 un{2. * rr.x / (z1.x + z2.x), 2. * rr.y / (z1.y + z2.y)};
  if ((h ? onB : onA) && 2 * l < K) {
    if (!(dl && (h ? rB : rA))) pst(p.ru_p + o, out, two);
    if (h ? rB : rA) {
      const d2 av{rs.x + (ra.x * invNs), rs.y + (ra.y * invNs)};
      if (!sa) {
        pst(p.ruAvg + o, av, two);
      } else {
        const d2 s2 = (sa & SA_FIRST) ? av : d2{av.x + sp.x, av.y + sp.y};
        pst(p.ruAvg_split + o, s2, two);
        if (sa & SA_LAST) pst(p.ruAvg + o, d2{s2.x * sa_inv, s2.y * sa_inv}, two);
      }
      pst(p.ru + o, rr, two);
      pst(p.u2 + o, un, two);
    } else if (fresh) {
      pst(p.ruAvg + o, ru, two);
    }
  }
  pack_rec_edge(upk, d, eA, eB, hasB, h, lc, (h ? onB : onA) && (h ? rB : rA) && 2 * l < K, two, un);
}

template <int NA, bool ODD = false, bool VROW = false>
__global__ __launch_bounds__(PAIR_THREADS) void k_scalars_edges_p(Dims d, Ptrs p) {
  const int eA = PAIR_EPW * pair_wave();
  if (eA >= d.nEdges) return;
  const bool hasB = PAIR_EPW == 2 && eA + 1 < d.nEdges;
  const int eB = hasB ? eA + 1 : eA;
  const int K = d.K, h = pair_half(), l = pair_lane(), ns = d.ns;
  const int lc = min(l, (ODD ? K + 1 : K) / 2 - 1);
  const bool two = !ODD || 2 * l + 1 < K;
  const int e = sel(h, eA, eB);
  const size_t o = (size_t)e * K + 2 * lc;
  const int na = sel(h, p.nAdvCellsForEdge[eA], p.nAdvCellsForEdge[eB]);
  __shared__ d2 wts[PAIR_WPB][PAIR_EPW][NA];
  d2 (&w)[NA] = wts[pair_row()][h];
  int ic[NA];
  double a[NA], b[NA];
  if constexpr (VROW) {
    if (l < NA) {
      const double aa = p.adv_coefs[(size_t)e * 15 + l], bb = p.adv_coefs_3rd[(size_t)e * 15 + l];
      w[l] = d2{aa + bb, aa - bb};
    }
    ld_row(p.advCellsForEdge + (size_t)e * 15, ic);
  } else {
#pragma unroll
    for (int j = 0; j < NA; ++j) {
      ic[j] = sel(h, p.advCellsForEdge[(size_t)eA * 15 + j], p.advCellsForEdge[(size_t)eB * 15 + j]);
      a[j] = sel(h, ld_uniform_f64(p.adv_coefs + (size_t)eA * 15 + j), ld_uniform_f64(p.adv_coefs + (size_t)eB * 15 + j));
      b[j] = sel(h, ld_uniform_f64(p.adv_coefs_3rd + (size_t)eA * 15 + j),
                 ld_uniform_f64(p.adv_coefs_3rd + (size_t)eB * 15 + j));
    }
  }
  auto wt = [&](int j, double sg, bool pos) -> double {
    if constexpr (VROW) {
      const d2 wj = w[j];
      return pos ? wj.x : wj.y;
    } else {
      return a[j] + sg * b[j];
    }
  };
  const d2 uh = ld2(p.ruAvg + o);
  const double sgx = sgn1(uh.x), sgy = sgn1(uh.y);
  const bool px = sgx > 0.0, py = sgy > 0.0;
  if constexpr (VROW) {
    pair_row_sync();
  }
  const bool hex = na == 10;
  bool st = (h == 0 || hasB) && 2 * l < K;
  const int bm = d.lbc ? sel(h, p.bdyMaskEdge[eA], p.bdyMaskEdge[eB]) : 0;
  if (bm >= N_RELAX_ZONE - 1) {
    if (bm > N_RELAX_ZONE) return;
    const double dv = sel(h, ld_uniform_f64(p.dvEdge + eA), ld_uniform_f64(p.dvEdge + eB));
    const int c1 = sel(h, p.cellsOnEdge[2 * eA], p.cellsOnEdge[2 * eB]);
    const int c2 = sel(h, p.cellsOnEdge[2 * eA + 1], p.cellsOnEdge[2 * eB + 1]);
    const double udx = copysign(0.5, uh.x), udy = copysign(0.5, uh.y);
    const d2 upos{dv * fabs(udx + 0.5), dv * fabs(udy + 0.5)}, uneg{dv * fabs(udx - 0.5), dv * fabs(udy - 0.5)};
    for (int is = 0; is < ns; ++is) {
      const d2 s1 = ld2(p.scalars2 + SIX(c1, 2 * lc, is)), s2 = ld2(p.scalars2 + SIX(c2, 2 * lc, is));
      if (st) pst(p.horiz_flux_array + HIX(e, 2 * lc, is), d2{upos.x * s1.x + uneg.x * s2.x, upos.y * s1.y + uneg.y * s2.y}, two);
    }
    return;
  }
  for (int is = 0; is < ns; ++is) {
    d2 sv[NA];
#pragma unroll
    for (int j = 0; j < NA; ++j) sv[j] = ld2(p.scalars2 + SIX(ic[j], 2 * lc, is));
    d2 acc{0.0, 0.0};
    if (hex) {
      acc.x = wt(0, sgx, px) * sv[0].x;
// ... 38 lines not shown
  if (on && 2 * l < K) pst(p.cqu + (size_t)e * K + 2 * lc, d2{1.0 / (1.0 + q.x), 1.0 / (1.0 + q.y)}, two);
}

struct MonoFlux2 {
  double *flux_arr, *flux_upwind_tmp, *flux_tmp;
};
template <int NA, bool ODD = false>
__global__ __launch_bounds__(PAIR_THREADS) void k_mono_edges1_p(Dims d, Ptrs p, int is, double dt, int nq = 1,
                                                                MonoFlux2 f2 = MonoFlux2{}) {
  __shared__ d2 wts[PAIR_WPB][PAIR_EPW][NA];
  const int eA = PAIR_EPW * pair_wave();
  if (eA >= d.nEdges) return;
  const bool hasB = PAIR_EPW == 2 && eA + 1 < d.nEdges;
  const int eB = hasB ? eA + 1 : eA;
  const int K = d.K, h = pair_half(), l = pair_lane(), ns = d.ns;
  const int lc = min(l, (ODD ? K + 1 : K) / 2 - 1);
  const bool two = !ODD || 2 * l + 1 < K;
  const int e = sel(h, eA, eB);
  const size_t o = (size_t)e * K + 2 * lc;
  const int2 ceA = *reinterpret_cast<const int2*>(p.cellsOnEdge + 2 * eA);
  const int2 ceB = *reinterpret_cast<const int2*>(p.cellsOnEdge + 2 * eB);
  const int na = sel(h, p.nAdvCellsForEdge[eA], p.nAdvCellsForEdge[eB]);
  d2 (&w)[NA] = wts[pair_row()][h];
  if (l < NA) {
    const double a = p.adv_coefs[(size_t)e * 15 + l], b = p.adv_coefs_3rd[(size_t)e * 15 + l];
    w[l] = d2{a + b, a - b};
  }
  int ic[NA];
  ld_row(p.advCellsForEdge + (size_t)e * 15, ic);
  const double dv = sel(h, ld_uniform_f64(p.dvEdge + eA), ld_uniform_f64(p.dvEdge + eB));
  const d2 uh = ld2(p.ruAvg + o);
  const int c1 = sel(h, ceA.x, ceB.x), c2 = sel(h, ceA.y, ceB.y);
  const bool on = c1 < d.nCellsSolve || c2 < d.nCellsSolve;
  const int bm = sel(h, p.bdyMaskEdge[eA], p.bdyMaskEdge[eB]);
  const bool upw = (d.lbc && bm == N_RELAX_ZONE) || bm == N_RELAX_ZONE - 1;
  pair_row_sync();
#pragma unroll 1
  for (int q = 0; q < nq; ++q) {
    const int iq = is + q;
    auto val = [&](const double* arr, int cc) {
      const d2 v = ld2(arr + SIX(cc, 2 * lc, iq));
      return cc < d.nCells ? v : d2{0.0, 0.0};
    };
    d2 sv[NA];
#pragma unroll
    for (int j = 0; j < NA; ++j) sv[j] = val(p.scalars2, ic[j]);
    const d2 so1 = val(p.scalars1, c1), so2 = val(p.scalars1, c2);
    d2 fa{0.0, 0.0};
    if (on) {
      if (na == 10) {
        const bool upx = uh.x > 0, upy = uh.y > 0;
        double ax = 0.0, ay = 0.0;
#pragma unroll
        for (int j = 0; j < 10 && j < NA; ++j) {
          const d2 wj = w[j];
          const double tx = (upx ? wj.x : wj.y) * sv[j].x, ty = (upy ? wj.x : wj.y) * sv[j].y;
          ax = (j == 0) ? tx : ax + tx;
          ay = (j == 0) ? ty : ay + ty;
        }
        fa = d2{uh.x * ax, uh.y * ay};
      } else {
        const bool px = sgn1(uh.x) > 0.0, py = sgn1(uh.y) > 0.0;
#pragma unroll
        for (int j = 0; j < NA; ++j) {
          if (j < na) {
            const d2 wj = w[j];
            fa.x = fa.x + (uh.x * (px ? wj.x : wj.y)) * sv[j].x;
            fa.y = fa.y + (uh.y * (py ? wj.x : wj.y)) * sv[j].y;
          }
        }
      }
    }
    d2 fu;
    fu.x = dv * dt * (fmax(0.0, uh.x) * so1.x + fmin(0.0, uh.x) * so2.x);
    fu.y = dv * dt * (fmax(0.0, uh.y) * so1.y + fmin(0.0, uh.y) * so2.y);
    if ((h == 0 || hasB) && 2 * l < K) {
      pst((q ? f2.flux_arr : p.flux_arr) + o, upw ? fu : fa, two);
      pst((q ? f2.flux_upwind_tmp : p.flux_upwind_tmp) + o, fu, two);
    }
  }
}

template <bool ODD = false>
__global__ __launch_bounds__(PAIR_THREADS) void k_vert_imp_coefs_p(Dims d, Ptrs p, double dts, double epssm) {
  const int K = d.K, h = pair_half(), l = pair_lane();
  const double dtseps = .5 * dts * (1. + epssm);
  const double rcv = RGAS / (CP - RGAS);
  const double c2 = CP * rcv;
  if (blockIdx.x == 0)
    for (int k = threadIdx.x; k < K; k += blockDim.x) p.cofrz[k] = dtseps * p.rdzw[k];
  const int cA = PAIR_EPW * pair_wave();
  if (cA >= d.nCellsSolve) return;
  const bool hasB = PAIR_EPW == 2 && cA + 1 < d.nCellsSolve;
  const int c = sel(h, cA, hasB ? cA + 1 : cA);
  const bool mine = h == 0 || hasB;
  const int lc = min(l, (ODD ? K + 1 : K) / 2 - 1);
  const bool two = !ODD || 2 * l + 1 < K;
  const int kx = 2 * l, ky = 2 * l + 1;
  const bool ax = kx < K, ay = ky < K;
  const size_t o = (size_t)c * K + 2 * lc;
  auto LDP = [&](const double* a) {
    d2 v = ld2(a + o);
    return d2{ax ? v.x : 0.0, ay ? v.y : 0.0};
  };
  auto LD1 = [&](const double* a) {
    d2 v = ld2(a + 2 * lc);
    return d2{ax ? v.x : 0.0, ay ? v.y : 0.0};
  };
  const d2 zz = LDP(p.zz), pp = LDP(p.exner), t = LDP(p.theta_m2), rb = LDP(p.rho_base), rtb = LDP(p.rtheta_base);
  const d2 pb = LDP(p.exner_base), rt = LDP(p.rtheta_p), cqw = LDP(p.cqw), qtot = LDP(p.qtot);
  const d2 fzm = LD1(p.fzm), fzp = LD1(p.fzp), rdzu = LD1(p.rdzu), rdzw = LD1(p.rdzw);
  const d2 zzm = km1(zz, l), pm = km1(pp, l), tm = km1(t, l);
  d2 cofwr{0.0, 0.0}, cofwz{0.0, 0.0}, coftz{0.0, 0.0}, cofwt{0.0, 0.0};
  auto lev1 = [&](bool act, int k, double zz_, double zzm_, double pp_, double pm_, double t_, double tm_,
                  double fzm_, double fzp_, double rdzu_, double cqw_, double& wr, double& wz, double& tz) {
    if (act && k >= 1) {
      wr = .5 * dtseps * GRAVITY * (fzm_ * zz_ + fzp_ * zzm_);
      wz = dtseps * c2 * (fzm_ * zz_ + fzp_ * zzm_) * rdzu_ * cqw_ * (fzm_ * pp_ + fzp_ * pm_);
      tz = dtseps * (fzm_ * t_ + fzp_ * tm_);
    }
  };
  lev1(ax, kx, zz.x, zzm.x, pp.x, pm.x, t.x, tm.x, fzm.x, fzp.x, rdzu.x, cqw.x, cofwr.x, cofwz.x, coftz.x);
  lev1(ay, ky, zz.y, zzm.y, pp.y, pm.y, t.y, tm.y, fzm.y, fzp.y, rdzu.y, cqw.y, cofwr.y, cofwz.y, coftz.y);
  if (ax) cofwt.x = .5 * dtseps * rcv * zz.x * GRAVITY * rb.x / (1. + qtot.x) * pp.x / ((rtb.x + rt.x) * pb.x);
  if (ay) cofwt.y = .5 * dtseps * rcv * zz.y * GRAVITY * rb.y / (1. + qtot.y) * pp.y / ((rtb.y + rt.y) * pb.y);
  const d2 coftz_p = kp1(coftz), coftz_m = km1(coftz, l), cofwt_m = km1(cofwt, l), rdzw_m = km1(rdzw, l);
  const d2 cofrz{dtseps * rdzw.x, dtseps * rdzw.y};
  const d2 cofrz_m = km1(cofrz, l);
  d2 a{0.0, 0.0}, b{1.0, 1.0}, cc{0.0, 0.0};
  auto lev2 = [&](bool act, int k, double& a_, double& b_, double& c_, double wz, double wr, double wt, double tz,
                  double tzm, double tzp, double wtm, double rw, double rwm, double z, double zm, double rz,
                  double rzm) {
    if (act && k >= 1) {
      a_ = -wz * tzm * rwm * zm + wr * rzm - wtm * tzm * rwm;
      b_ = 1. + wz * (tz * rw * z + tz * rwm * zm) - tz * (wt * rw - wtm * rwm) + wr * (rz - rzm);
      c_ = -wz * tzp * rw * z - wr * rz + wt * tzp * rw;
    }
  };
  lev2(ax, kx, a.x, b.x, cc.x, cofwz.x, cofwr.x, cofwt.x, coftz.x, coftz_m.x, coftz_p.x, cofwt_m.x, rdzw.x,
       rdzw_m.x, zz.x, zzm.x, cofrz.x, cofrz_m.x);
  lev2(ay, ky, a.y, b.y, cc.y, cofwz.y, cofwr.y, cofwt.y, coftz.y, coftz_m.y, coftz_p.y, cofwt_m.y, rdzw.y,
       rdzw_m.y, zz.y, zzm.y, cofrz.y, cofrz_m.y);
  const bool fx = kx >= 1 && ax, fy = ay;
  d2 alpha{0.0, 0.0}, gamma{0.0, 0.0};
  for (int it = 0; it < (ODD ? K + 1 : K) / 2; ++it) {
    const double gpx = lane_shr1(gamma.y);
    if (fx) {
      alpha.x = 1. / (b.x - a.x * (l == 0 ? 0.0 : gpx));
      gamma.x = cc.x * alpha.x;
    }
    if (fy) {
      alpha.y = 1. / (b.y - a.y * gamma.x);
      gamma.y = cc.y * alpha.y;
    }
  }
  if (mine && ax) {
    if (l == 0) {
      p.cofwr[o + 1] = cofwr.y;
      p.cofwz[o + 1] = cofwz.y;
    } else {
      pst(p.cofwr + o, cofwr, two);
      pst(p.cofwz + o, cofwz, two);
    }
    pst(p.cofwt + o, cofwt, two);
    pst(p.a_tri + o, a, two);
    pst(p.alpha_tri + o, alpha, two);
    pst(p.gamma_tri + o, gamma, two);
  }
  if (mine && kx <= K) {
    double* ct = p.coftz + (size_t)c * (K + 1) + kx;
    if (ky <= K) {
      ct[0] = coftz.x;
      ct[1] = coftz.y;
    } else {
      ct[0] = coftz.x;
    }
  }
}

template <bool DD, bool UP = false, bool ODD = false>
__global__ __launch_bounds__(PAIR_THREADS) void k_acoustic_edges_p(Dims d, Ptrs p, double dts, int small_step,
                                                                   double coef_divdamp, int phase, int fresh,
                                                                   UnpackMap um = UnpackMap{}) {
  int eA, eB;
  bool hasB;
  if (!pair_edges(d, p, phase, eA, eB, hasB)) return;
  const int K = d.K, h = pair_half(), l = pair_lane();
  const bool lev = 2 * l < K;
  const int lc = min(l, (ODD ? K + 1 : K) / 2 - 1);
  const bool two = !ODD || 2 * l + 1 < K;
  const int e = sel(h, eA, eB);
  const size_t o = (size_t)e * K + 2 * lc;
  const int2 ceA = *reinterpret_cast<const int2*>(p.cellsOnEdge + 2 * eA);
  const int2 ceB = *reinterpret_cast<const int2*>(p.cellsOnEdge + 2 * eB);
  const int bA = phase ? p.edge_bnd[eA] : 0, bB = phase ? p.edge_bnd[eB] : 0;
  const d2 tu = ld2(p.tend_u + o);
  auto active = [&](int2 ce, int bnd) {
    return (ce.x < d.nCellsSolve || ce.y < d.nCellsSolve) && !(phase && ((bnd != 0) != (phase == 2)));
  };
  const bool onA = active(ceA, bA), onB = hasB && active(ceB, bB);
  if (!onA && !onB) return;
  const bool st = lev && (h ? onB : onA);
  if (small_step == 1) {
    const d2 rup = {dts * tu.x, dts * tu.y};
    if (st) {
      pst(p.ru_p + o, rup, two);
      pst(p.ruAvg + o, rup, two);
    }
    return;
  }
  d2 rup, rua;
  if (fresh) {
    rup = d2{dts * tu.x, dts * tu.y};
    rua = rup;
  } else {
    rup = ld2(p.ru_p + o);
    rua = ld2(p.ruAvg + o);
  }
  const d2 cqu = ld2(p.cqu + o), zxu = ld2(p.zxu + o);
  const double mask = sel(h, ld_uniform_f64(p.specZoneMaskEdge + eA), ld_uniform_f64(p.specZoneMaskEdge + eB));
  const double invDc = sel(h, ld_uniform_f64(p.invDcEdge + eA), ld_uniform_f64(p.invDcEdge + eB));
  const int c1 = sel(h, ceA.x, ceB.x), c2 = sel(h, ceA.y, ceB.y);
  const size_t o1 = (size_t)c1 * K + 2 * lc, o2 = (size_t)c2 * K + 2 * lc;
  const d2 rt1 = UP ? ld_pp<ODD>(d, p, um, 0, c1, lc, st) : ld2(p.rtheta_pp + o1);
  const d2 rt2 = UP ? ld_pp<ODD>(d, p, um, 0, c2, lc, st) : ld2(p.rtheta_pp + o2);
  const d2 zz1 = ld2(p.zz + o1), zz2 = ld2(p.zz + o2), ex1 = ld2(p.exner + o1), ex2 = ld2(p.exner + o2);
  const d2 rp1 = UP ? ld_pp<ODD>(d, p, um, 1, c1, lc, st) : ld2(p.rho_pp + o1);
  const d2 rp2 = UP ? ld_pp<ODD>(d, p, um, 1, c2, lc, st) : ld2(p.rho_pp + o2);
  d2 ro1{}, ro2{}, th1{}, th2{};
  if (DD) {
    ro1 = ld2(p.rtheta_pp_old + o1);
    ro2 = ld2(p.rtheta_pp_old + o2);
    th1 = ld2(p.theta_m1 + o1);
    th2 = ld2(p.theta_m1 + o2);
  }
  const double rcv = RGAS / (CP - RGAS);
  const double c2v = CP * rcv;
  auto level = [&](double r, double tu_, double cq, double zx, double a1, double a2, double z1, double z2,
                   double x1, double x2, double p1, double p2, double o1_, double o2_, double t1, double t2) {
    if (DD) {
      const double dd1 = -(a1 - o1_);
      const double dd2 = -(a2 - o2_);
      r = r + coef_divdamp * (dd2 - dd1) * (1.0 - mask) / (t1 + t2);
    }
    double pgrad = ((a2 - a1) * invDc) / (.5 * (z2 + z1));
    pgrad = cq * 0.5 * c2v * (x1 + x2) * pgrad;
    pgrad = pgrad + 0.5 * zx * GRAVITY * (p1 + p2);
    return r + dts * (tu_ - (1.0 - mask) * pgrad);
  };
  rup.x = level(rup.x, tu.x, cqu.x, zxu.x, rt1.x, rt2.x, zz1.x, zz2.x, ex1.x, ex2.x, rp1.x, rp2.x, ro1.x, ro2.x,
// ... 16 lines not shown
  r.rtps = p.rtheta_p_save[o];
  r.rtb = p.rtheta_base[o];
  r.exb = rk_step == 3 ? p.exner_base[o] : 0.0;
  r.rtd = (rk_step == 3 && d.diabatic) ? p.rt_diabatic_tend[o] : 0.0;
  return r;
}
__device__ __forceinline__ void recover_cell_fused(const Dims& d, const Ptrs& p, int c, int k, double zz_k, double rws,
                                                   double fzm_k, double fzp_k, const RecIn& ri, double rhopp,
                                                   double rtpp, double rwp, double wwa, double dt, double invNs,
                                                   int rk_step, int sa, double sa_inv) {
  const int K = d.K;
  const size_t K1 = K + 1;
  const bool act = k < K;
  const int kc = min(k, K - 1), kw = min(k, K);
  const size_t o = (size_t)c * K + kc, ow = (size_t)c * K1 + kw;
  const double rcv = RGAS / (CP - RGAS);
  const double rps = ri.rps, rb = ri.rb, rtps = ri.rtps, rtb = ri.rtb;
  const double fzm = act ? fzm_k : 0.0, fzp = act ? fzp_k : 0.0;
  const double zz = act ? zz_k : 0.0, zzm = up1(zz);
  double rz = 0.0;
  if (act) {
    const double rho_p = rps + rhopp;
    if (rk_step == 3) p.rho_p[o] = rho_p;
    rz = rho_p + rb;
    p.rho_zz2[o] = rz;
  }
  double w = 0.0;
  if (act && k >= 1) {
    store_avg(p.wwAvg, p.wwAvg_split, ow, rws + (wwa * invNs), sa, sa_inv);
    const double rw = rws + rwp;
    p.rw[ow] = rw;
    w = rw / (fzm * zz + fzp * zzm);
  }
  if (k <= K) p.w2[ow] = w;
  if (act) {
    if (rk_step == 3) {
      const double rtp = rtps + rtpp - dt * rz * ri.rtd;
      p.rtheta_p[o] = rtp;
      p.theta_m2[o] = (rtp + rtb) / rz;
      const double ex = pow(zz * (RGAS / P0) * (rtp + rtb), rcv);
      p.exner[o] = ex;
      p.pressure_p[o] = zz * RGAS * (ex * rtp + rtb * (ex - ri.exb));
    } else {
      const double rtp = rtps + rtpp;
      p.rtheta_p[o] = rtp;
      p.theta_m2[o] = (rtp + rtb) / rz;
    }
  }
}

__device__ __forceinline__ void pack_column(const PackMap& pk, int c, int k, bool act, double rt, double rho) {
  if (!pk.start) return;
  const int s0 = __builtin_amdgcn_readfirstlane(pk.start[c]), s1 = __builtin_amdgcn_readfirstlane(pk.start[c + 1]);
  for (int s = s0; s < s1; ++s) {
    if (act) pk.rt[s][k] = rt;
    if (act && pk.rho) pk.rho[s][k] = rho;
  }
}

__device__ __forceinline__ void pack_rec_cell(const XPack& pk, int c, int k, bool act, bool actw, double rw,
                                              double rho, double rt) {
  if (!pk.start) return;
  const int s0 = __builtin_amdgcn_readfirstlane(pk.start[c]), s1 = __builtin_amdgcn_readfirstlane(pk.start[c + 1]);
  for (int s = s0; s < s1; ++s) {
    const int f = __builtin_amdgcn_readfirstlane(pk.fid[s]);
    double* dst = pk.dst[s];
    if (f == 0) {
      if (actw) dst[k] = rw;
    } else if (act) {
      dst[k] = f == 1 ? rho : rt;
    }
  }
}

template <int ME>
struct AcIn {
  int ne;
  double sdv[ME], invA, spec;
  double rtpp, rhopp, rwp, wwa;
  double thc, trho, tth, tw, ru[ME], th[ME];
  double coftz, zz, cofwt, cofwz, cofwr, a_tri, alpha_tri, gamma_tri;
  double rz, dss, rws, rw, w2, cofrz, rdzw, fzm, fzp;
};
template <int ME>
__device__ __forceinline__ void load_ac_own(const Ptrs& p, size_t o, size_t ow, int kc, AcIn<ME>& in) {
  in.trho = p.tend_rho[o];
  in.coftz = p.coftz[ow], in.cofwt = p.cofwt[o], in.cofwz = p.cofwz[o], in.cofwr = p.cofwr[o];
  in.a_tri = p.a_tri[o], in.alpha_tri = p.alpha_tri[o], in.gamma_tri = p.gamma_tri[o];
  in.dss = p.dss[o];
  in.cofrz = p.cofrz[kc];
}
template <int ME, bool FIN>
__device__ __forceinline__ void acoustic_cells_col(const Dims& d, const Ptrs& p, int c, const AcIn<ME>& in, double dts,
                                                   int small_step, double epssm, double rdt, double invNs, int rk_step,
                                                   int keep_pp, const PackMap& pk, int dl, const XPack& rp, int sa = 0,
                                                   double sa_inv = 0.0) {
  const int k = lane_id(), K = d.K;
  const bool act = k < K, actw = k <= K;
  const int kc = min(k, K - 1), kw = min(k, K);
  const size_t K1 = K + 1;
  const size_t o = (size_t)c * K + kc, ow = (size_t)c * K1 + kw;
  const int ne = in.ne;
  const double invA = in.invA, spec = in.spec;
  double rtpp = in.rtpp, rhopp = in.rhopp, rwp = in.rwp, wwa = in.wwa;
  const double thc = in.thc, trho = in.trho, tth = in.tth, tw = in.tw;
  const double coftz = in.coftz, zz = in.zz, cofwt = in.cofwt, cofwz = in.cofwz, cofwr = in.cofwr;
  const double a_tri = in.a_tri, alpha_tri = in.alpha_tri, gamma_tri = in.gamma_tri;
  const double rz = in.rz, dss = in.dss, rws = in.rws, rw = in.rw, w2 = in.w2;
  const double cofrz = in.cofrz, rdzw = in.rdzw, fzm = in.fzm, fzp = in.fzp;
  RecIn ri{};
  const double rtpp_old = (small_step == 1) ? 0.0 : rtpp;
  const double resm = (1.0 - epssm) / (1.0 + epssm);
  if (small_step == 1) { wwa = 0.0; rhopp = 0.0; rtpp = 0.0; rwp = 0.0; }
  if (!act) { rhopp = 0.0; rtpp = 0.0; }
  if (spec == 0.0) {
    double ts = 0.0, rs = 0.0;
#pragma unroll
    for (int i = 0; i < ME; ++i) {
      if (i < ne) {
        const double flux = dts * in.sdv[i] * in.ru[i] * invA;
        rs = rs - flux;
        ts = ts - flux * 0.5 * (in.th[i] + thc);
      }
    }
    double dn2[2] = {coftz, rwp};
    col_shift(dn2, 1);
    const double coftz_p = dn2[0], rwp_p = dn2[1];
    if (act) {
      rs = rhopp + dts * trho + rs - cofrz * resm * (rwp_p - rwp);
      ts = rtpp + dts * tth + ts - resm * rdzw * (coftz_p * rwp_p - coftz * rwp);
    }
    if (act && k >= 1) wwa = wwa + 0.5 * (1.0 - epssm) * rwp;
    double up7[7] = {zz, ts, rs, rtpp, rhopp, cofwt, rz};
    col_shift(up7, -1);
    const double zzm = up7[0], tsm = up7[1], rsm = up7[2], rtppm = up7[3], rhoppm = up7[4], cofwtm = up7[5];
    if (act && k >= 1) {
      rwp = rwp + dts * tw - cofwz * ((zz * ts - zzm * tsm) + resm * (zz * rtpp - zzm * rtppm)) -
            cofwr * ((rs + rsm) + resm * (rhopp + rhoppm)) + cofwt * (ts + resm * rtpp) +
            cofwtm * (tsm + resm * rtppm);
    }
#ifdef MPAS_WIDE
    rwp = column_solve(rwp, a_tri, alpha_tri, gamma_tri, k, K);
#else
    rwp = thomas_column(rwp, a_tri, alpha_tri, gamma_tri, k, K);
#endif
    const double rzm = up7[6];
    if (act && k >= 1) {
      const double dd = rws - rw;
      rwp = (rwp + dd - dts * dss * (fzm * zz + fzp * zzm) * (fzm * rz + fzp * rzm) * w2) / (1.0 + dts * dss) - dd;
      wwa = wwa + 0.5 * (1.0 + epssm) * rwp;
    }
    const double rwp_p2 = dn1(rwp);
    const double rho_new = rs - cofrz * (rwp_p2 - rwp);
    const double rt_new = ts - rdzw * (coftz_p * rwp_p2 - coftz * rwp);
    if (act) {
      if (FIN && dl) {
        p.rtheta_pp_old[o] = rt_new - rtpp_old;
      } else {
        p.rtheta_pp_old[o] = rtpp_old;
        p.rtheta_pp[o] = rt_new;
      }
      if (!FIN || keep_pp) p.rho_pp[o] = rho_new;
    }
    if (actw) {
      if (!FIN || keep_pp) p.rw_p[ow] = rwp;
      if (!FIN) p.wwAvg[ow] = wwa;
      else if (k == 0 || k == K) store_avg(p.wwAvg, p.wwAvg_split, ow, wwa, sa, sa_inv);
    }
    pack_column(pk, c, k, act, rt_new, rho_new);
    if (FIN) pack_rec_cell(rp, c, k, act, actw, rwp, rho_new, rt_new);
    if (FIN) ri = load_rec_in(d, p, o, rk_step);
    if (FIN) recover_cell_fused(d, p, c, k, zz, rws, fzm, fzp, ri, rho_new, rt_new, rwp, wwa, rdt, invNs, rk_step, sa, sa_inv);
  } else {
    if (act) {
      rhopp = rhopp + dts * trho;
      rtpp = rtpp + dts * tth;
      rwp = rwp + dts * tw;
      wwa = wwa + 0.5 * (1.0 + epssm) * rwp;
      if (FIN && dl) {
        p.rtheta_pp_old[o] = rtpp - rtpp_old;
      } else {
        p.rtheta_pp_old[o] = rtpp_old;
        p.rtheta_pp[o] = rtpp;
      }
      p.rho_pp[o] = rhopp;
    }
    if (actw) {
      p.rw_p[ow] = rwp;
      if (!FIN) p.wwAvg[ow] = wwa;
      else if (k == 0 || k == K) store_avg(p.wwAvg, p.wwAvg_split, ow, wwa, sa, sa_inv);
    }
    pack_column(pk, c, k, act, rtpp, rhopp);
    if (FIN) pack_rec_cell(rp, c, k, act, actw, rwp, rhopp, rtpp);
    if (FIN) ri = load_rec_in(d, p, o, rk_step);
    if (FIN) recover_cell_fused(d, p, c, k, zz, rws, fzm, fzp, ri, rhopp, rtpp, rwp, wwa, rdt, invNs, rk_step, sa, sa_inv);
  }
}

#if defined(MPAS_WIDE) && WIDE_THREADS == 320
#define ACOUSTIC_CELLS_ATTR __attribute__((amdgpu_waves_per_eu(FIN ? 4 : 5)))
#else
#define ACOUSTIC_CELLS_ATTR
#endif
template <int ME, bool FIN = false>
__global__ __launch_bounds__(BLOCK_THREADS) ACOUSTIC_CELLS_ATTR void k_acoustic_cells_r(Dims d, Ptrs p, double dts, int small_step,
                                                                    double epssm, double rdt = 0.0,
                                                                    double invNs = 0.0, int rk_step = 0,
                                                                    int keep_pp = 1, PackMap pk = PackMap{}, int dl = 0,
                                                                    XPack rp = XPack{}, int sa = 0, double sa_inv = 0.0) {
  const int c = wave_elem(0);
  if (c >= d.nCells) return;
  const int k = lane_id(), K = d.K;
  const bool act = k < K, actw = k <= K;
  const int kc = min(k, K - 1), kw = min(k, K);
  const size_t K1 = K + 1;
  const size_t o = (size_t)c * K + kc, ow = (size_t)c * K1 + kw;
  const bool first = small_step == 1;
  double rtpp = first ? 0.0 : p.rtheta_pp[o];
  if (c >= d.nCellsSolve) {
    if (act) p.rtheta_pp_old[o] = (FIN && dl) ? rtpp - (first ? 0.0 : rtpp) : (first ? 0.0 : rtpp);
    return;
  }
  AcIn<ME> in;
  int re[ME], rc[ME];
#pragma unroll
  for (int i = 0; i < ME; ++i) {
    re[i] = p.cell_rec[(size_t)c * CELL_REC + i];
    rc[i] = p.cell_rec[(size_t)c * CELL_REC + CELL_REC_ME + i];
    in.sdv[i] = ld_uniform_f64(p.cell_sdv + (size_t)c * ME + i);
  }
  in.ne = p.cell_rec[(size_t)c * CELL_REC + 14];
  in.invA = FIN ? p.invAreaCell[c] : ld_uniform_f64(p.invAreaCell + c);
  in.spec = FIN ? p.specZoneMaskCell[c] : ld_uniform_f64(p.specZoneMaskCell + c);
  in.rtpp = rtpp;
  in.rhopp = first ? 0.0 : p.rho_pp[o], in.rwp = first ? 0.0 : p.rw_p[ow], in.wwa = first ? 0.0 : p.wwAvg[ow];
  in.thc = p.theta_m1[o], in.trho = p.tend_rho[o], in.tth = p.tend_theta[o], in.tw = p.tend_w[ow];
  const double* __restrict__ rusrc = small_step == 1 ? p.tend_u : p.ru_p;
#pragma unroll
  for (int i = 0; i < ME; ++i) {
    in.ru[i] = rusrc[(size_t)re[i] * K + kc];
    in.th[i] = p.theta_m1[(size_t)rc[i] * K + kc];
  }
  if (small_step == 1) {
#pragma unroll
    for (int i = 0; i < ME; ++i) in.ru[i] = dts * in.ru[i];
  }
  in.coftz = p.coftz[ow], in.zz = p.zz[o], in.cofwt = p.cofwt[o], in.cofwz = p.cofwz[o], in.cofwr = p.cofwr[o];
  in.a_tri = p.a_tri[o], in.alpha_tri = p.alpha_tri[o], in.gamma_tri = p.gamma_tri[o];
  in.rz = p.rho_zz2_rd[o], in.dss = p.dss[o], in.rws = p.rw_save[ow], in.rw = p.rw_rd[ow], in.w2 = p.w2_rd[ow];
  in.cofrz = p.cofrz[kc], in.rdzw = p.rdzw[kc], in.fzm = p.fzm[kc], in.fzp = p.fzp[kc];
  acoustic_cells_col<ME, FIN>(d, p, c, in, dts, small_step, epssm, rdt, invNs, rk_step, keep_pp, pk, dl, rp, sa, sa_inv);
}

#ifndef MPAS_WIDE
struct TendAcArgs {
  double dts, epssm, rdt, invNs;
  int rk_step, keep_pp, dl, store_tend;
  int sa;
  double sa_inv;
};
template <int ME, bool RK1, bool FIN>
__global__ __launch_bounds__(BLOCK_THREADS) void k_dyn_cells3_acoustic_r(Dims d, Ptrs p, Config cf, DynTendScal s,
                                                                         TendAcArgs a) {
  const int c = wave_elem(0);
  if (c >= d.nCells) return;
  const int k = lane_id(), K = d.K;
  const int kc = min(k, K - 1), kw = min(k, K);
  const size_t o = (size_t)c * K + kc, ow = (size_t)c * (K + 1) + kw;
  if (c >= d.nCellsSolve) {
    if (k < K) p.rtheta_pp_old[o] = 0.0;
    return;
  }
  TendCarry<ME> cy;
  dyn_cells3_col<ME, RK1, true, true>(d, p, cf, s, TendRd{p.ru_rd, p.rw_rd, p.w2_rd, p.rho_zz2_rd, p.theta_m2_rd}, c,
                                      a.store_tend != 0, cy);
  AcIn<ME> in;
  load_ac_own(p, o, ow, kc, in);
  if (RK1) {
#pragma unroll
    for (int i = 0; i < ME; ++i) cy.thn[i] = p.theta_m1[(size_t)cy.co[i] * K + kc];
  }
  in.spec = ld_uniform_f64(p.specZoneMaskCell + c);
  in.ne = cy.ne;
  in.invA = cy.invA;
  in.rtpp = in.rhopp = in.rwp = in.wwa = 0.0;
  in.thc = cy.thc, in.tth = cy.tth, in.tw = cy.tw;
#pragma unroll
  for (int i = 0; i < ME; ++i) {
    in.sdv[i] = cy.sdv[i];
    in.ru[i] = a.dts * cy.ut[i];
    in.th[i] = cy.thn[i];
  }
  in.zz = cy.zz, in.rz = cy.rz, in.rws = cy.rws, in.rw = cy.rw, in.w2 = cy.w2;
  in.rdzw = cy.rdzw, in.fzm = cy.fzm, in.fzp = cy.fzp;
  acoustic_cells_col<ME, FIN>(d, p, c, in, a.dts, 1, a.epssm, a.rdt, a.invNs, a.rk_step, a.keep_pp, PackMap{}, a.dl,
                              XPack{}, a.sa, a.sa_inv);
}
#endif

__global__ __launch_bounds__(BLOCK_THREADS) void k_acoustic_cells(Dims d, Ptrs p, double dts, int small_step, double epssm) {
  const int c = wave_elem(0);
  if (c >= d.nCells) return;
  const int k = lane_id(), K = d.K;
  const bool act = k < K, actw = k <= K;
  const size_t K1 = K + 1;
  const size_t o = (size_t)c * K + k, ow = (size_t)c * K1 + k;
  double rtpp = LD(p.rtheta_pp, o);
  if (act) p.rtheta_pp_old[o] = (small_step == 1) ? 0.0 : rtpp;
  if (c >= d.nCellsSolve) return;
  const double resm = (1.0 - epssm) / (1.0 + epssm);
  double rhopp = LD(p.rho_pp, o), rwp = LDW(p.rw_p, ow), wwa = LDW(p.wwAvg, ow);
  if (small_step == 1) { wwa = 0.0; rhopp = 0.0; rtpp = 0.0; rwp = 0.0; }
  if (p.specZoneMaskCell[c] == 0.0) {
    double ts = 0.0, rs = 0.0;
    const int ne = p.nEdgesOnCell[c];
    const double invA = p.invAreaCell[c];
    const double thc = LD(p.theta_m1, o);
    for (int i = 0; i < ne; ++i) {
      const int e = uni(p.edgesOnCell[c * d.maxEdges + i]);
      const int c1 = p.cellsOnEdge[2 * e], c2 = p.cellsOnEdge[2 * e + 1];
      if (act) {
        const double rue = small_step == 1 ? dts * p.tend_u[(size_t)e * K + k] : p.ru_p[(size_t)e * K + k];
        const double flux = p.edgesOnCell_sign[c * d.maxEdges + i] * dts * p.dvEdge[e] * rue * invA;
        rs = rs - flux;
        const double th1 = (c1 == c) ? thc : p.theta_m1[(size_t)c1 * K + k];
        const double th2 = (c2 == c) ? thc : p.theta_m1[(size_t)c2 * K + k];
        ts = ts - flux * 0.5 * (th2 + th1);
      }
    }
    const double cofrz = act ? p.cofrz[k] : 0.0, rdzw = act ? p.rdzw[k] : 0.0;
    const double coftz = LDW(p.coftz, ow), coftz_p = dn1(coftz);
    const double rwp_p = dn1(rwp);
    if (act) {
      rs = rhopp + dts * p.tend_rho[o] + rs - cofrz * resm * (rwp_p - rwp);
      ts = rtpp + dts * p.tend_theta[o] + ts - resm * rdzw * (coftz_p * rwp_p - coftz * rwp);
    }
    if (act && k >= 1) wwa = wwa + 0.5 * (1.0 - epssm) * rwp;
    const double zz = LD(p.zz, o), zzm = up1(zz);
    const double tsm = up1(ts), rsm = up1(rs), rtppm = up1(rtpp), rhoppm = up1(rhopp);
    const double cofwt = LD(p.cofwt, o), cofwtm = up1(cofwt);
    if (act && k >= 1) {
      rwp = rwp + dts * p.tend_w[ow] -
            p.cofwz[o] * ((zz * ts - zzm * tsm) + resm * (zz * rtpp - zzm * rtppm)) -
            p.cofwr[o] * ((rs + rsm) + resm * (rhopp + rhoppm)) + cofwt * (ts + resm * rtpp) +
            cofwtm * (tsm + resm * rtppm);
    }
    const double a_tri = LD(p.a_tri, o), alpha_tri = LD(p.alpha_tri, o), gamma_tri = LD(p.gamma_tri, o);
#ifdef MPAS_WIDE
    rwp = column_solve(rwp, a_tri, alpha_tri, gamma_tri, k, K);
#else
    for (int kk = 1; kk < K; ++kk) {
      const double xm = readlane_d(rwp, kk - 1);
      if (k == kk) rwp = (rwp - a_tri * xm) * alpha_tri;
    }
    for (int kk = K - 1; kk >= 0; --kk) {
      const double xp = readlane_d(rwp, kk + 1);
      if (k == kk) rwp = rwp - gamma_tri * xp;
    }
#endif
    if (act && k >= 1) {
      const double fzm = p.fzm[k], fzp = p.fzp[k];
      const double rz = p.rho_zz2_rd[o], rzm = p.rho_zz2_rd[o - 1];
      const double dss = p.dss[o];
      const double dd = p.rw_save[ow] - p.rw_rd[ow];
      rwp = (rwp + dd - dts * dss * (fzm * zz + fzp * zzm) * (fzm * rz + fzp * rzm) * p.w2_rd[ow]) / (1.0 + dts * dss) - dd;
      wwa = wwa + 0.5 * (1.0 + epssm) * rwp;
    }
    const double rwp_p2 = dn1(rwp);
    if (act) {
      p.rho_pp[o] = rs - cofrz * (rwp_p2 - rwp);
      p.rtheta_pp[o] = ts - rdzw * (coftz_p * rwp_p2 - coftz * rwp);
    }
    if (actw) {
      p.rw_p[ow] = rwp;
      p.wwAvg[ow] = wwa;
    }
  } else {
    if (act) {
      rhopp = rhopp + dts * p.tend_rho[o];
// ... 1345 lines not shown
```

### mpas-model_amd/mpas_dycore/dycore.py

```python
from __future__ import annotations

import ctypes as C

import numpy as np

from . import _lib
from . import fields as F
from .layout import LOC_N, to_fortran

STATE_INPUTS = ("u", "w", "scalars")
MODEL_INIT_OUT = ("invAreaCell", "invDvEdge", "invDcEdge", "invAreaTriangle", "edgesOnVertex_sign",
                  "edgesOnCell_sign", "zb_cell", "zb3_cell", "kiteForCell", "nAdvCellsForEdge", "advCellsForEdge",
                  "adv_coefs", "adv_coefs_3rd", "meshScalingDel2", "meshScalingDel4", "meshScalingRegionalCell",
                  "meshScalingRegionalEdge", "dss")
MODEL_INIT_IN = ("deriv_two", "zb", "zb3", "meshDensity", "areaCell", "areaTriangle")
RECONSTRUCT_IN = ("xCell", "yCell", "zCell", "xEdge", "yEdge", "zEdge")
DIAG_INPUTS = ("theta", "rho", "rho_base", "theta_base")
_SKIP = set(STATE_INPUTS) | set(DIAG_INPUTS) | {"xCell", "yCell", "zCell", "xEdge", "yEdge", "zEdge", "xVertex",
                                                "yVertex", "zVertex",
                                                "latVertex", "lonVertex", "areaCell", "areaTriangle",
                                                "meshDensity", "indexToCellID", "deriv_two", "zb", "zb3",
                                                "w_velocity_max", "wind_speed_level1_max", "updraft_helicity_max",
                                                *F.MICROP_FIELD}

# ... 338 lines not shown
            self.microphysics(dt, time_level)
        finally:
            self._check(self.lib.mpas_dyc_set_profile(self.h, 0), "set_profile")
        out = (C.c_double * 8)()
        self._check(self.lib.mpas_dyc_get_profile(self.h, out, 8), "get_profile")
        return float(out[7])

    def finish_step(self, dt: float):
        self._check(self.lib.mpas_dyc_finish_step(self.h, float(dt)), "finish_step")

    def output_diagnostics(self, time_level: int = 1):
        self._check(self.lib.mpas_dyc_output_diagnostics(self.h, int(time_level)), "output_diagnostics")

    def set_summary(self, global_minmax_vel: bool = True, detailed_minmax_vel: bool = False,
                    global_minmax_sca: bool = False):
        flags = ((_lib.PRINT_GLOBAL_MINMAX_VEL if global_minmax_vel else 0)
                 | (_lib.PRINT_DETAILED_MINMAX_VEL if detailed_minmax_vel else 0)
                 | (_lib.PRINT_GLOBAL_MINMAX_SCA if global_minmax_sca else 0))
        self._check(self.lib.mpas_dyc_set_summary(self.h, flags), "set_summary")

    def summarize_timestep(self, log=None, block: int | None = None) -> dict:
        s = _lib.Summary()
        mm = (C.c_double * (2 * self.ns))()
        if block is None:
            rc = self.lib.mpas_dyc_get_summary(self.h, C.byref(s), mm, 2 * self.ns)
        else:
            rc = self.lib.mpas_dyc_get_block_summary(self.h, int(block), C.byref(s), mm, 2 * self.ns)
        self._check(rc, "summarize_timestep")
        out = {"flags": s.flags, "w_min": s.w_min, "w_max": s.w_max, "u_min": s.u_min, "u_max": s.u_max,
               "nan_w": s.nan_w, "nan_u": s.nan_u, "scalars": [(mm[2 * i], mm[2 * i + 1]) for i in range(self.ns)]}
        for n in ("w_min_at", "w_max_at", "u_min_at", "u_max_at", "wsp_max_at"):
            e = getattr(s, n)
            out[n] = {"value": e.value, "k": e.k, "index": e.index, "lat": e.lat, "lon": e.lon}
        lines = []
        if s.flags & _lib.PRINT_DETAILED_MINMAX_VEL:
            lines.append("")
            for n, tag in (("w_min_at", "min w"), ("w_max_at", "max w"), ("u_min_at", "min u"),
                           ("u_max_at", "max u"), ("wsp_max_at", "max wsp")):
                e = out[n]
                lines.append(f" global {tag}: {e['value']} k={e['k']}, {e['lat']} lat, {e['lon']} lon")
        elif s.flags & _lib.PRINT_GLOBAL_MINMAX_VEL:
            lines += ["", f"global min, max w {s.w_min} {s.w_max}", f"global min, max u {s.u_min} {s.u_max}"]
        if s.flags & _lib.PRINT_GLOBAL_MINMAX_SCA:
            if not s.flags & (_lib.PRINT_GLOBAL_MINMAX_VEL | _lib.PRINT_DETAILED_MINMAX_VEL):
                lines.append("")
            lines += [f" global min, max scalar {i + 1} {a} {b}" for i, (a, b) in enumerate(out["scalars"])]
        out["log"] = lines
        if log is not None:
            for ln in lines:
                log(ln)
        if s.flags & _lib.PRINT_DETAILED_MINMAX_VEL and (s.nan_w or s.nan_u):
            raise DycoreError("NaN detected in '" + ("w" if s.nan_w else "u") + "' field.")
        return out

    def shift_time_levels(self):
        self._check(self.lib.mpas_dyc_shift_time_levels(self.h), "shift_time_levels")

    def synchronize(self):
        self._check(self.lib.mpas_dyc_synchronize(self.h), "synchronize")

    def use_graph(self, on: bool = True):
        self._check(self.lib.mpas_dyc_use_graph(self.h, 1 if on else 0), "use_graph")

    def time_acoustic_step(self, dts: float, small_step: int = 2, reps: int = 10):
        ms = C.c_double()
        ks = (C.c_double * 3)()
        self._check(self.lib.mpas_dyc_time_acoustic_step(self.h, float(dts), int(small_step), int(reps),
                                                         C.byref(ms), ks), "time_acoustic_step")
        return ms.value, list(ks)

    def layout(self, block: int = 0) -> dict:
        out = (C.c_int32 * 4)()
        self._check(self.lib.mpas_dyc_block_layout(self.h, int(block), out), "block_layout")
        return {"maxEdges": out[0], "maxEdges2": out[1], "family": ("general", "batched", "pair")[out[2]],
                "column": ("wavefront", "wide", "wide256", "wide512", "wide192", "wide320", "wide384",
                           "wide448")[out[3]]}

    def fused_tend_acoustic(self) -> tuple:
        m = int(self.lib.mpas_dyc_fused_tend_acoustic(self.h))
        return tuple(rk for rk in (1, 2, 3) if m & (1 << (rk - 1)))

    def folded_passes(self) -> tuple:
        m = int(self.lib.mpas_dyc_folded_passes(self.h))
        return tuple(n for i, n in enumerate(("substep_avg", "rk1_edges", "recover_diag")) if m & (1 << i))

    def exchange_profile(self, dt: float, itimestep: int = 1) -> dict:
        self._check(self.lib.mpas_dyc_set_profile(self.h, 1), "set_profile")
        try:
            self.atm_timestep(dt, itimestep)
        finally:
            self._check(self.lib.mpas_dyc_set_profile(self.h, 0), "set_profile")
        out = (C.c_double * 5)()
        self._check(self.lib.mpas_dyc_get_profile(self.h, out, 5), "get_profile")
        return {"exchanges": int(out[0]), "ms_step_eager": out[1], "ms_exchange_exposed": out[2],
                "ms_compute": out[1] - out[2], "rccl_groups": int(out[3]), "ms_rccl_groups": out[4]}

    def last_exchange(self) -> str:
        k = self.lib.mpas_dyc_last_exchange(self.h) if self.h else None
        return k.decode() if k else ""

    @staticmethod
    def rccl_version() -> int:
        return int(_lib.load().mpas_dyc_rccl_version())

    def acoustic_bytes(self) -> float:
        return self.lib.mpas_dyc_acoustic_bytes(self.h)

    def close(self):
        if getattr(self, "h", None):
            self.lib.mpas_dyc_destroy(self.h)
            self.h = None

    def __del__(self):
        try:
            self.close()
        except Exception:
            pass


_LOCS = {}
for _n in ("theta_m", "rho_zz", "rho_p", "rtheta_p", "exner", "pressure_p", "pressure", "kdiff", "ke", "divergence", "rw",
           "wwAvg", "cqw", "h_divergence", "pv_cell", "rho_pp", "rtheta_pp", "rw_p", "exner_base", "pressure_base",
           "rtheta_base", "coftz", "cofwz", "cofwr", "cofwt", "a_tri", "alpha_tri", "gamma_tri", "rw_save",
           "tend_rtheta_adv", "rho_p_save", "rtheta_p_save", "rho_zz_old_split", "rtheta_pp_old", "wwAvg_split",
           "tend_rtheta_physics", "tend_rho_physics", "rqvdynten",
           "scalars_tend", "rthdynten", "rt_diabatic_tend", "theta_euler", "w_euler", "uReconstructX",
           "uReconstructY", "uReconstructZ", "uReconstructZonal", "uReconstructMeridional"):
    _LOCS[_n] = "cell"
for _n in ("ru", "ruAvg", "ru_p", "ru_save", "cqu", "rho_edge", "v", "pv_edge", "gradPVn", "gradPVt", "tend_ru_physics",
           "ruAvg_split", "u_euler"):
    _LOCS[_n] = "edge"
for _n in ("vorticity", "pv_vertex"):
    _LOCS[_n] = "vertex"


def _loc_of(pool: str, name: str):
    if pool == "tend" and name == "u":
        return "edge"
    if name in _LOCS:
        return _LOCS[name]
    return F.LOCATION.get(name)
```

Baseline: 266.6 million cell-updates/s.

## Derive implicit-solver coefficients in acoustic kernels and skip unused stage-average stores

The acoustic cell kernels now recompute cofwr, a_tri and gamma_tri on the fly from coefficients they already load, so the vertical-implicit coefficient kernel can skip storing those three arrays when it is not the last call. Without this, those arrays are written once and reread on every acoustic substep. Separately, the ruAvg stores in RK stages 1 and 2 are skipped with a new SA_SKIP flag when the split transport does not consume them. Both cut HBM traffic in exchange for extra arithmetic and state tracking (vic_own, invalidated when a coefficient field is touched externally). Storage is still done on the final call so external readers see valid arrays.

```diff
diff --git a/mpas-model_amd/csrc/dycore.hip b/mpas-model_amd/csrc/dycore.hip
--- a/mpas-model_amd/csrc/dycore.hip
+++ b/mpas-model_amd/csrc/dycore.hip
@@ -173,6 +173,10 @@
   bool overlap_all = false;
   bool fuse_tend_acoustic = true;
   bool fold_substep_avg = true;
+  bool skip_stage_avg = true;
+  bool derive_coefs = true;
+  bool vic_own = false;
+  double vic_dtseps = 0.0;
   bool fold_rk1_edges = true;
   bool fuse_recover_diag = true;
   std::vector<XField> late_fs;
@@ -844,19 +848,38 @@
 }
 
 
-void vert_imp_coefs(mpas_dyc_ctx* ctx, const Dims& d, const Ptrs& p, double dts) {
+bool fused_recover(const Dims& d) { return batched(d) && (d.maxEdges == 6 || d.maxEdges == 7); }
+
+bool coefs_derived(const mpas_dyc_ctx* ctx, const Dims& d) {
+#ifdef MPAS_WIDE
+  return false;
+#else
+  return ctx->derive_coefs && ctx->vic_own && g_vic != 2 && fused_recover(d);
+#endif
+}
+void coefs_touched(mpas_dyc_ctx* ctx, const Field& f) {
+  if (f.pool != "diag") return;
+  for (const char* n : {"coftz", "cofwz", "cofwr", "cofwt", "a_tri", "alpha_tri", "gamma_tri", "cofrz"})
+    if (f.name == n) ctx->vic_own = false;
+}
+
+void vert_imp_coefs(mpas_dyc_ctx* ctx, const Dims& d, const Ptrs& p, double dts, bool last = true) {
+  if (!ctx->planning) {
+    ctx->vic_own = true;
+    ctx->vic_dtseps = .5 * dts * (1. + ctx->cf.epssm);
+  }
+  const int store_drv = (last || !coefs_derived(ctx, d)) ? 1 : 0;
   if (g_vic == 2) {
     LAUNCH(k_vert_imp_coefs<true>, std::max(d.nCellsSolve, 1), d, p, dts, ctx->cf.epssm);
     if (d.nCellsSolve > 0 && !ctx->planning)
       hipLaunchKernelGGL(k_vert_imp_lu, dim3((unsigned)((d.nCellsSolve + 63) / 64)), dim3(64), 0, ctx->stream, d, p);
   } else if (pair_layout(d) && g_vic == 1) {
-    LAUNCH_PE((k_vert_imp_coefs_p<false>), (k_vert_imp_coefs_p<true>), std::max(d.nCellsSolve, 1), d, p, dts, ctx->cf.epssm);
+    LAUNCH_PE((k_vert_imp_coefs_p<false>), (k_vert_imp_coefs_p<true>), std::max(d.nCellsSolve, 1), d, p, dts, ctx->cf.epssm,
+              store_drv);
   } else {
     LAUNCH(k_vert_imp_coefs<false>, std::max(d.nCellsSolve, 1), d, p, dts, ctx->cf.epssm);
   }
 }
-
-bool fused_recover(const Dims& d) { return batched(d) && (d.maxEdges == 6 || d.maxEdges == 7); }
 
 struct TendAcoustic {
   Ptrs pf;
@@ -865,6 +888,7 @@
   int keep_pp, dl, store_tend;
   int sa;
   double sa_inv;
+  bool drv;
 };
 bool tend_acoustic_fused(const mpas_dyc_ctx* ctx, int rk_step, int nsub) {
 #ifdef MPAS_WIDE
@@ -880,6 +904,17 @@
   return false;
 #else
   if (!ctx->fold_substep_avg || needs_exchange(ctx) || ctx->lbc || ctx->blk.size() != 1) return false;
+  if (!ctx->cf.split_dynamics_transport) return false;
+  const Dims& d = ctx->blk[0].d;
+  return pair_layout(d) && fused_recover(d) && d.nCellsSolve == d.nCells && d.nEdgesSolve == d.nEdges &&
+         d.n_bnd_edges == 0;
+#endif
+}
+bool stage_avg_skipped(const mpas_dyc_ctx* ctx) {
+#ifdef MPAS_WIDE
+  return false;
+#else
+  if (!ctx->skip_stage_avg || needs_exchange(ctx) || ctx->lbc || ctx->blk.size() != 1) return false;
   if (!ctx->cf.split_dynamics_transport) return false;
   const Dims& d = ctx->blk[0].d;
   return pair_layout(d) && fused_recover(d) && d.nCellsSolve == d.nCells && d.nEdgesSolve == d.nEdges &&
@@ -1005,8 +1040,17 @@
 #ifndef MPAS_WIDE
   if (ta) {
     const TendAcArgs a{ta->dts, cf.epssm, ta->rdt, ta->invNs, rk_step, ta->keep_pp, ta->dl,
-                       ta->store_tend, ta->sa, ta->sa_inv};
+                       ta->store_tend, ta->sa, ta->sa_inv, ctx->vic_dtseps};
     const bool m6 = d.maxEdges == 6, fin = ta->fin;
+    if (ta->drv) {
+      if (m6 && rk_step == 1) LAUNCH((k_dyn_cells3_acoustic_r<6, true, true, AC_DRV>), d.nCells, d, ta->pf, cf, s, a);
+      if (m6 && rk_step != 1 && fin) LAUNCH((k_dyn_cells3_acoustic_r<6, false, true, AC_DRV>), d.nCells, d, ta->pf, cf, s, a);
+      if (m6 && rk_step != 1 && !fin) LAUNCH((k_dyn_cells3_acoustic_r<6, false, false, AC_DRV>), d.nCells, d, ta->pf, cf, s, a);
+      if (!m6 && rk_step == 1) LAUNCH((k_dyn_cells3_acoustic_r<7, true, true, AC_DRV>), d.nCells, d, ta->pf, cf, s, a);
+      if (!m6 && rk_step != 1 && fin) LAUNCH((k_dyn_cells3_acoustic_r<7, false, true, AC_DRV>), d.nCells, d, ta->pf, cf, s, a);
+      if (!m6 && rk_step != 1 && !fin) LAUNCH((k_dyn_cells3_acoustic_r<7, false, false, AC_DRV>), d.nCells, d, ta->pf, cf, s, a);
+      return;
+    }
     if (m6 && rk_step == 1) LAUNCH((k_dyn_cells3_acoustic_r<6, true, true>), d.nCells, d, ta->pf, cf, s, a);
     if (m6 && rk_step != 1 && fin) LAUNCH((k_dyn_cells3_acoustic_r<6, false, true>), d.nCells, d, ta->pf, cf, s, a);
     if (m6 && rk_step != 1 && !fin) LAUNCH((k_dyn_cells3_acoustic_r<6, false, false>), d.nCells, d, ta->pf, cf, s, a);
@@ -1077,6 +1121,25 @@
 void acoustic_cells(mpas_dyc_ctx* ctx, const Dims& d, const Ptrs& p, double dts, int small_step, int fin = 0,
                     double rdt = 0.0, double invNs = 0.0, int rk_step = 0, int keep_pp = 1, PackMap pk = PackMap{},
                     int dl = 0, XPack rp = XPack{}, int sa = 0, double sa_inv = 0.0) {
+#ifndef MPAS_WIDE
+  if (coefs_derived(ctx, d)) {
+    const double cds = ctx->vic_dtseps, eps = ctx->cf.epssm;
+    const bool m6 = d.maxEdges == 6;
+    if (m6 && fin)
+      LAUNCH((k_acoustic_cells_r<6, true, AC_DRV>), d.nCells, d, p, dts, small_step, eps, rdt, invNs, rk_step, keep_pp, pk, dl,
+             rp, sa, sa_inv, cds);
+    else if (m6)
+      LAUNCH((k_acoustic_cells_r<6, false, AC_DRV>), d.nCells, d, p, dts, small_step, eps, 0.0, 0.0, 0, 1, pk, 0, XPack{}, 0,
+             0.0, cds);
+    else if (fin)
+      LAUNCH((k_acoustic_cells_r<7, true, AC_DRV>), d.nCells, d, p, dts, small_step, eps, rdt, invNs, rk_step, keep_pp, pk, dl,
+             rp, sa, sa_inv, cds);
+    else
+      LAUNCH((k_acoustic_cells_r<7, false, AC_DRV>), d.nCells, d, p, dts, small_step, eps, 0.0, 0.0, 0, 1, pk, 0, XPack{}, 0,
+             0.0, cds);
+    return;
+  }
+#endif
   if (batched(d) && d.maxEdges == 6) {
     if (fin)
       LAUNCH((k_acoustic_cells_r<6, true>), d.nCells, d, p, dts, small_step, ctx->cf.epssm, rdt, invNs, rk_step, keep_pp,
@@ -1434,11 +1497,13 @@
   }
   if (ctx->overlap_all) sml_fused = false, rec_overlap = true;
   const bool avg_folded = substep_avg_folded(ctx);
+  const bool avg_skipped = stage_avg_skipped(ctx);
   const bool rd_fused = recover_diag_fused(ctx);
-  EACHV(Ppre, vert_imp_coefs(ctx, d, p, rk_sub_timestep[0]));
+  const bool o3 = cf.time_integration_order == 3;
+  EACHV(Ppre, vert_imp_coefs(ctx, d, p, rk_sub_timestep[0], !o3 && dynamics_split == 1));
   for (int dynamics_substep = 1; dynamics_substep <= dynamics_split; ++dynamics_substep) {
     for (int rk_step = 1; rk_step <= 3; ++rk_step) {
-      if (cf.time_integration_order == 3 && rk_step == 2) EACH(vert_imp_coefs(ctx, d, p, rk_sub_timestep[1]));
+      if (o3 && rk_step == 2) EACH(vert_imp_coefs(ctx, d, p, rk_sub_timestep[1], dynamics_substep == dynamics_split));
       const bool last_stage = dynamics_substep == dynamics_split && rk_step == 3;
       const bool hdiv_next = !lbc && rk_step < 3 && (!split || (rk_step == 1 && cf.time_integration_order == 3));
       const std::vector<Ptrs>& PS = rk_step == 1 ? Ppre : P;
@@ -1452,13 +1517,13 @@
       const bool fuse_ta = tend_acoustic_fused(ctx, rk_step, nsub);
       const int sa = (avg_folded && rk_step == 3)
                          ? SA_ON | (dynamics_substep == 1 ? SA_FIRST : 0) | (dynamics_substep == dynamics_split ? SA_LAST : 0)
-                         : 0;
+                         : (avg_skipped && rk_step < 3) ? SA_SKIP : 0;
       const double sa_inv = 1.0 / (double)dynamics_split;
       TendAcoustic ta{};
       if (fuse_ta)
         ta = TendAcoustic{PF[0], nsub == 1, dts, rk_timestep[rk_step - 1], 1 / (double)nsub, last_stage ? 1 : 0,
                           nsub == 1 ? damping_delta(ctx, ctx->blk[0].d, last_stage) : 0, (nsub > 1 || last_stage) ? 1 : 0,
-                          nsub == 1 ? sa : 0, sa_inv};
+                          nsub == 1 ? sa : 0, sa_inv, coefs_derived(ctx, ctx->blk[0].d)};
       const TendAcoustic* tap = fuse_ta ? &ta : nullptr;
       if (pending) {
         EACHV(PS, dyn_tend(ctx, d, p, rk_step, dt, 1, hdiv_prev && batched(d)));
@@ -1592,7 +1657,7 @@
         if (rk_step == 3 && dynamics_substep < dynamics_split) {
           CHK((exchange)(ctx, {{"state", "theta_m", 2, ALL_LAYERS}, {"diag", "pressure_p", 0, ALL_LAYERS},
                                {"diag", "rtheta_p", 0, ALL_LAYERS}, {"diag", "exner", 0, ALL_LAYERS}}));
-          EACH(vert_imp_coefs(ctx, d, p, rk_sub_timestep[0]));
+          EACH(vert_imp_coefs(ctx, d, p, rk_sub_timestep[0], !o3 && dynamics_substep + 1 == dynamics_split));
         }
       } else if (rk_step < 3) {
         CHK(xchg(xd));
@@ -1601,7 +1666,7 @@
         xd.insert(xd.end(), {{"state", "theta_m", 2, ALL_LAYERS}, {"diag", "pressure_p", 0, ALL_LAYERS},
                              {"diag", "rtheta_p", 0, ALL_LAYERS}, {"diag", "exner", 0, ALL_LAYERS}});
         CHK(xchg(xd));
-        EACH(vert_imp_coefs(ctx, d, p, rk_sub_timestep[0]));
+        EACH(vert_imp_coefs(ctx, d, p, rk_sub_timestep[0], !o3 && dynamics_substep + 1 == dynamics_split));
         CHK(xwait());
       } else if (split) {
         CHK(exchange_async(ctx, xd));
@@ -1939,6 +2004,8 @@
   if (const char* oa = getenv("MPAS_DYCORE_OVERLAP_ALL")) ctx->overlap_all = std::string(oa) == "1";
   if (const char* ft = getenv("MPAS_DYCORE_FUSE_TEND_ACOUSTIC")) ctx->fuse_tend_acoustic = std::string(ft) != "0";
   if (const char* fs = getenv("MPAS_DYCORE_FOLD_SUBSTEP_AVG")) ctx->fold_substep_avg = std::string(fs) != "0";
+  if (const char* dc = getenv("MPAS_DYCORE_DERIVE_COEFS")) ctx->derive_coefs = std::string(dc) != "0";
+  if (const char* ss = getenv("MPAS_DYCORE_SKIP_STAGE_AVG")) ctx->skip_stage_avg = std::string(ss) != "0";
   if (const char* fe = getenv("MPAS_DYCORE_FOLD_RK1_EDGES")) ctx->fold_rk1_edges = std::string(fe) != "0";
   if (const char* fr = getenv("MPAS_DYCORE_FUSE_RECOVER_DIAG")) ctx->fuse_recover_diag = std::string(fr) != "0";
   if (const char* ov = getenv("MPAS_DYCORE_OVERLAP")) ctx->overlap = std::atoi(ov);
@@ -2042,6 +2109,7 @@
   Field* f = find(*b, pool, name);
   if (!f) return nullptr;
   if (f->me || (f->pool == "mesh" && (f->name == "zb_cell" || f->name == "zb3_cell"))) ctx->bnd_ready = false;
+  coefs_touched(ctx, *f);
   return f->buf[slot_of(ctx, *f, time_level)];
 }
 
@@ -2082,6 +2150,7 @@
     CHK(f->group == G_ON_SET ? alloc_field(ctx, b, *f, false)
                              : alloc_group(ctx, f->group, GROUPS[f->group].all_blocks ? nullptr : &b));
   if (f->me) ctx->bnd_ready = false;
+  coefs_touched(ctx, *f);
   if (f->is_int && f->target != T_NONE) {
     const int64_t n = field_elems(b, *f);
     std::vector<int32_t> tmp(n);
@@ -3058,6 +3127,10 @@
   for (const auto& b : ctx->blk) all = all && rk1_edge_folded(ctx, b.d);
   if (all) m |= 2;
   if (recover_diag_fused(ctx)) m |= 4;
+  if (stage_avg_skipped(ctx)) m |= 8;
+  bool drv = !ctx->blk.empty();
+  for (const auto& b : ctx->blk) drv = drv && coefs_derived(ctx, b.d);
+  if (drv) m |= 16;
   return m;
 }
 
diff --git a/mpas-model_amd/csrc/kernels.hip b/mpas-model_amd/csrc/kernels.hip
--- a/mpas-model_amd/csrc/kernels.hip
+++ b/mpas-model_amd/csrc/kernels.hip
@@ -359,6 +359,17 @@
   for (int iq = d.moist_start; iq <= d.moist_end; ++iq)
     qtotal = qtotal + 0.5 * (p.scalars2[SIX(c1, k, iq)] + p.scalars2[SIX(c2, k, iq)]);
   p.cqu[(size_t)e * K + k] = 1.0 / (1.0 + qtotal);
+}
+
+__device__ __forceinline__ double vic_cofwr(double dtseps, double fzm, double fzp, double zz, double zzm) {
+  return .5 * dtseps * GRAVITY * (fzm * zz + fzp * zzm);
+}
+__device__ __forceinline__ double vic_a(double wz, double wr, double wtm, double tzm, double rwm, double zm,
+                                        double rzm) {
+  return -wz * tzm * rwm * zm + wr * rzm - wtm * tzm * rwm;
+}
+__device__ __forceinline__ double vic_c(double wz, double wr, double wt, double tzp, double rw, double z, double rz) {
+  return -wz * tzp * rw * z - wr * rz + wt * tzp * rw;
 }
 
 template <bool SPLIT = false>
@@ -381,7 +392,7 @@
   const double zzm = up1(zz), pm = up1(pp), tm = up1(t);
   double cofwr = 0.0, cofwz = 0.0, coftz = 0.0;
   if (act && k >= 1) {
-    cofwr = .5 * dtseps * GRAVITY * (fzm * zz + fzp * zzm);
+    cofwr = vic_cofwr(dtseps, fzm, fzp, zz, zzm);
     cofwz = dtseps * c2 * (fzm * zz + fzp * zzm) * rdzu * cqw * (fzm * pp + fzp * pm);
     coftz = dtseps * (fzm * t + fzp * tm);
   }
@@ -392,10 +403,10 @@
   const double cofrz = dtseps * rdzw, cofrz_m = up1(cofrz);
   double a = 0.0, b = 1.0, cc = 0.0;
   if (act && k >= 1) {
-    a = -cofwz * coftz_m * rdzw_m * zzm + cofwr * cofrz_m - cofwt_m * coftz_m * rdzw_m;
+    a = vic_a(cofwz, cofwr, cofwt_m, coftz_m, rdzw_m, zzm, cofrz_m);
     b = 1. + cofwz * (coftz * rdzw * zz + coftz * rdzw_m * zzm) - coftz * (cofwt * rdzw - cofwt_m * rdzw_m) +
         cofwr * (cofrz - cofrz_m);
-    cc = -cofwz * coftz_p * rdzw * zz - cofwr * cofrz + cofwt * coftz_p * rdzw;
+    cc = vic_c(cofwz, cofwr, cofwt, coftz_p, rdzw, zz, cofrz);
   }
   double alpha = 0.0, gamma = 0.0;
 #ifdef MPAS_WIDE
@@ -2589,8 +2600,9 @@
   return ld2(fld + o);
 }
 
-enum { SA_ON = 1, SA_FIRST = 2, SA_LAST = 4 };
+enum { SA_ON = 1, SA_FIRST = 2, SA_LAST = 4, SA_SKIP = 8 };
 __device__ __forceinline__ void store_avg(double* avg, double* split, size_t i, double a, int sa, double inv) {
+  if (sa & SA_SKIP) return;
   if (!sa) {
     avg[i] = a;
     return;
@@ -2658,7 +2670,7 @@
   const bool rB = onB && (phase ? bB : p.edge_bnd[eB]) == 0;
   const d2 rs = ld2(p.ru_save + o);
   const d2 ra = fresh ? ru : ld2(p.ruAvg + o);
-  const d2 sp = (sa && !(sa & SA_FIRST)) ? ld2(p.ruAvg_split + o) : d2{0.0, 0.0};
+  const d2 sp = ((sa & SA_ON) && !(sa & SA_FIRST)) ? ld2(p.ruAvg_split + o) : d2{0.0, 0.0};
   const d2 z1 = ld2(p.rho_zz2 + o1), z2 = ld2(p.rho_zz2 + o2);
   const d2 rr{rs.x + out.x, rs.y + out.y};
   const d2 un{2. * rr.x / (z1.x + z2.x), 2. * rr.y / (z1.y + z2.y)};
@@ -2666,7 +2678,8 @@
     if (!(dl && (h ? rB : rA))) pst(p.ru_p + o, out, two);
     if (h ? rB : rA) {
       const d2 av{rs.x + (ra.x * invNs), rs.y + (ra.y * invNs)};
-      if (!sa) {
+      if (sa & SA_SKIP) {
+      } else if (!sa) {
         pst(p.ruAvg + o, av, two);
       } else {
         const d2 s2 = (sa & SA_FIRST) ? av : d2{av.x + sp.x, av.y + sp.y};
@@ -2871,7 +2884,8 @@
 }
 
 template <bool ODD = false>
-__global__ __launch_bounds__(PAIR_THREADS) void k_vert_imp_coefs_p(Dims d, Ptrs p, double dts, double epssm) {
+__global__ __launch_bounds__(PAIR_THREADS) void k_vert_imp_coefs_p(Dims d, Ptrs p, double dts, double epssm,
+                                                                   int store_drv = 1) {
   const int K = d.K, h = pair_half(), l = pair_lane();
   const double dtseps = .5 * dts * (1. + epssm);
   const double rcv = RGAS / (CP - RGAS);
@@ -2904,7 +2918,7 @@
   auto lev1 = [&](bool act, int k, double zz_, double zzm_, double pp_, double pm_, double t_, double tm_,
                   double fzm_, double fzp_, double rdzu_, double cqw_, double& wr, double& wz, double& tz) {
     if (act && k >= 1) {
-      wr = .5 * dtseps * GRAVITY * (fzm_ * zz_ + fzp_ * zzm_);
+      wr = vic_cofwr(dtseps, fzm_, fzp_, zz_, zzm_);
       wz = dtseps * c2 * (fzm_ * zz_ + fzp_ * zzm_) * rdzu_ * cqw_ * (fzm_ * pp_ + fzp_ * pm_);
       tz = dtseps * (fzm_ * t_ + fzp_ * tm_);
     }
@@ -2921,9 +2935,9 @@
                   double tzm, double tzp, double wtm, double rw, double rwm, double z, double zm, double rz,
                   double rzm) {
     if (act && k >= 1) {
-      a_ = -wz * tzm * rwm * zm + wr * rzm - wtm * tzm * rwm;
+      a_ = vic_a(wz, wr, wtm, tzm, rwm, zm, rzm);
       b_ = 1. + wz * (tz * rw * z + tz * rwm * zm) - tz * (wt * rw - wtm * rwm) + wr * (rz - rzm);
-      c_ = -wz * tzp * rw * z - wr * rz + wt * tzp * rw;
+      c_ = vic_c(wz, wr, wt, tzp, rw, z, rz);
     }
   };
   lev2(ax, kx, a.x, b.x, cc.x, cofwz.x, cofwr.x, cofwt.x, coftz.x, coftz_m.x, coftz_p.x, cofwt_m.x, rdzw.x,
@@ -2945,16 +2959,18 @@
   }
   if (mine && ax) {
     if (l == 0) {
-      p.cofwr[o + 1] = cofwr.y;
+      if (store_drv) p.cofwr[o + 1] = cofwr.y;
       p.cofwz[o + 1] = cofwz.y;
     } else {
-      pst(p.cofwr + o, cofwr, two);
+      if (store_drv) pst(p.cofwr + o, cofwr, two);
       pst(p.cofwz + o, cofwz, two);
     }
     pst(p.cofwt + o, cofwt, two);
-    pst(p.a_tri + o, a, two);
     pst(p.alpha_tri + o, alpha, two);
-    pst(p.gamma_tri + o, gamma, two);
+    if (store_drv) {
+      pst(p.a_tri + o, a, two);
+      pst(p.gamma_tri + o, gamma, two);
+    }
   }
   if (mine && kx <= K) {
     double* ct = p.coftz + (size_t)c * (K + 1) + kx;
@@ -3137,19 +3153,22 @@
   double coftz, zz, cofwt, cofwz, cofwr, a_tri, alpha_tri, gamma_tri;
   double rz, dss, rws, rw, w2, cofrz, rdzw, fzm, fzp;
 };
-template <int ME>
+template <int ME, int DRV = 0>
 __device__ __forceinline__ void load_ac_own(const Ptrs& p, size_t o, size_t ow, int kc, AcIn<ME>& in) {
   in.trho = p.tend_rho[o];
-  in.coftz = p.coftz[ow], in.cofwt = p.cofwt[o], in.cofwz = p.cofwz[o], in.cofwr = p.cofwr[o];
-  in.a_tri = p.a_tri[o], in.alpha_tri = p.alpha_tri[o], in.gamma_tri = p.gamma_tri[o];
+  in.coftz = p.coftz[ow], in.cofwt = p.cofwt[o], in.cofwz = p.cofwz[o], in.alpha_tri = p.alpha_tri[o];
+  in.cofwr = (DRV & 1) ? 0.0 : p.cofwr[o];
+  in.a_tri = (DRV & 2) ? 0.0 : p.a_tri[o];
+  in.gamma_tri = (DRV & 4) ? 0.0 : p.gamma_tri[o];
   in.dss = p.dss[o];
   in.cofrz = p.cofrz[kc];
 }
-template <int ME, bool FIN>
+constexpr int AC_DRV = 7;
+template <int ME, bool FIN, int DRV = 0>
 __device__ __forceinline__ void acoustic_cells_col(const Dims& d, const Ptrs& p, int c, const AcIn<ME>& in, double dts,
                                                    int small_step, double epssm, double rdt, double invNs, int rk_step,
                                                    int keep_pp, const PackMap& pk, int dl, const XPack& rp, int sa = 0,
-                                                   double sa_inv = 0.0) {
+                                                   double sa_inv = 0.0, double cdtseps = 0.0) {
   const int k = lane_id(), K = d.K;
   const bool act = k < K, actw = k <= K;
   const int kc = min(k, K - 1), kw = min(k, K);
@@ -3159,8 +3178,8 @@
   const double invA = in.invA, spec = in.spec;
   double rtpp = in.rtpp, rhopp = in.rhopp, rwp = in.rwp, wwa = in.wwa;
   const double thc = in.thc, trho = in.trho, tth = in.tth, tw = in.tw;
-  const double coftz = in.coftz, zz = in.zz, cofwt = in.cofwt, cofwz = in.cofwz, cofwr = in.cofwr;
-  const double a_tri = in.a_tri, alpha_tri = in.alpha_tri, gamma_tri = in.gamma_tri;
+  const double coftz = in.coftz, zz = in.zz, cofwt = in.cofwt, cofwz = in.cofwz, alpha_tri = in.alpha_tri;
+  double cofwr = in.cofwr, a_tri = in.a_tri, gamma_tri = in.gamma_tri;
   const double rz = in.rz, dss = in.dss, rws = in.rws, rw = in.rw, w2 = in.w2;
   const double cofrz = in.cofrz, rdzw = in.rdzw, fzm = in.fzm, fzp = in.fzp;
   RecIn ri{};
@@ -3189,10 +3208,18 @@
     double up7[7] = {zz, ts, rs, rtpp, rhopp, cofwt, rz};
     col_shift(up7, -1);
     const double zzm = up7[0], tsm = up7[1], rsm = up7[2], rtppm = up7[3], rhoppm = up7[4], cofwtm = up7[5];
+    if (DRV & 1) cofwr = (act && k >= 1) ? vic_cofwr(cdtseps, fzm, fzp, zz, zzm) : 0.0;
     if (act && k >= 1) {
       rwp = rwp + dts * tw - cofwz * ((zz * ts - zzm * tsm) + resm * (zz * rtpp - zzm * rtppm)) -
             cofwr * ((rs + rsm) + resm * (rhopp + rhoppm)) + cofwt * (ts + resm * rtpp) +
             cofwtm * (tsm + resm * rtppm);
+    }
+    if (DRV & 6) {
+      const double coftz_m = up1(coftz), rdzw_m = up1(rdzw);
+      if (DRV & 2)
+        a_tri = (act && k >= 1) ? vic_a(cofwz, cofwr, cofwtm, coftz_m, rdzw_m, zzm, cdtseps * rdzw_m) : 0.0;
+      if (DRV & 4)
+        gamma_tri = (act && k >= 1) ? vic_c(cofwz, cofwr, cofwt, coftz_p, rdzw, zz, cdtseps * rdzw) * alpha_tri : 0.0;
     }
 #ifdef MPAS_WIDE
     rwp = column_solve(rwp, a_tri, alpha_tri, gamma_tri, k, K);
@@ -3257,12 +3284,13 @@
 #else
 #define ACOUSTIC_CELLS_ATTR
 #endif
-template <int ME, bool FIN = false>
+template <int ME, bool FIN = false, int DRV = 0>
 __global__ __launch_bounds__(BLOCK_THREADS) ACOUSTIC_CELLS_ATTR void k_acoustic_cells_r(Dims d, Ptrs p, double dts, int small_step,
                                                                     double epssm, double rdt = 0.0,
                                                                     double invNs = 0.0, int rk_step = 0,
                                                                     int keep_pp = 1, PackMap pk = PackMap{}, int dl = 0,
-                                                                    XPack rp = XPack{}, int sa = 0, double sa_inv = 0.0) {
+                                                                    XPack rp = XPack{}, int sa = 0, double sa_inv = 0.0,
+                                                                    double cdtseps = 0.0) {
   const int c = wave_elem(0);
   if (c >= d.nCells) return;
   const int k = lane_id(), K = d.K;
@@ -3300,11 +3328,14 @@
 #pragma unroll
     for (int i = 0; i < ME; ++i) in.ru[i] = dts * in.ru[i];
   }
-  in.coftz = p.coftz[ow], in.zz = p.zz[o], in.cofwt = p.cofwt[o], in.cofwz = p.cofwz[o], in.cofwr = p.cofwr[o];
-  in.a_tri = p.a_tri[o], in.alpha_tri = p.alpha_tri[o], in.gamma_tri = p.gamma_tri[o];
+  in.coftz = p.coftz[ow], in.zz = p.zz[o], in.cofwt = p.cofwt[o], in.cofwz = p.cofwz[o], in.alpha_tri = p.alpha_tri[o];
+  in.cofwr = (DRV & 1) ? 0.0 : p.cofwr[o];
+  in.a_tri = (DRV & 2) ? 0.0 : p.a_tri[o];
+  in.gamma_tri = (DRV & 4) ? 0.0 : p.gamma_tri[o];
   in.rz = p.rho_zz2_rd[o], in.dss = p.dss[o], in.rws = p.rw_save[ow], in.rw = p.rw_rd[ow], in.w2 = p.w2_rd[ow];
   in.cofrz = p.cofrz[kc], in.rdzw = p.rdzw[kc], in.fzm = p.fzm[kc], in.fzp = p.fzp[kc];
-  acoustic_cells_col<ME, FIN>(d, p, c, in, dts, small_step, epssm, rdt, invNs, rk_step, keep_pp, pk, dl, rp, sa, sa_inv);
+  acoustic_cells_col<ME, FIN, DRV>(d, p, c, in, dts, small_step, epssm, rdt, invNs, rk_step, keep_pp, pk, dl, rp, sa,
+                                   sa_inv, cdtseps);
 }
 
 #ifndef MPAS_WIDE
@@ -3313,8 +3344,9 @@
   int rk_step, keep_pp, dl, store_tend;
   int sa;
   double sa_inv;
+  double cdtseps;
 };
-template <int ME, bool RK1, bool FIN>
+template <int ME, bool RK1, bool FIN, int DRV = 0>
 __global__ __launch_bounds__(BLOCK_THREADS) void k_dyn_cells3_acoustic_r(Dims d, Ptrs p, Config cf, DynTendScal s,
                                                                          TendAcArgs a) {
   const int c = wave_elem(0);
@@ -3330,7 +3362,7 @@
   dyn_cells3_col<ME, RK1, true, true>(d, p, cf, s, TendRd{p.ru_rd, p.rw_rd, p.w2_rd, p.rho_zz2_rd, p.theta_m2_rd}, c,
                                       a.store_tend != 0, cy);
   AcIn<ME> in;
-  load_ac_own(p, o, ow, kc, in);
+  load_ac_own<ME, DRV>(p, o, ow, kc, in);
   if (RK1) {
 #pragma unroll
     for (int i = 0; i < ME; ++i) cy.thn[i] = p.theta_m1[(size_t)cy.co[i] * K + kc];
@@ -3348,8 +3380,8 @@
   }
   in.zz = cy.zz, in.rz = cy.rz, in.rws = cy.rws, in.rw = cy.rw, in.w2 = cy.w2;
   in.rdzw = cy.rdzw, in.fzm = cy.fzm, in.fzp = cy.fzp;
-  acoustic_cells_col<ME, FIN>(d, p, c, in, a.dts, 1, a.epssm, a.rdt, a.invNs, a.rk_step, a.keep_pp, PackMap{}, a.dl,
-                              XPack{}, a.sa, a.sa_inv);
+  acoustic_cells_col<ME, FIN, DRV>(d, p, c, in, a.dts, 1, a.epssm, a.rdt, a.invNs, a.rk_step, a.keep_pp, PackMap{}, a.dl,
+                                   XPack{}, a.sa, a.sa_inv, a.cdtseps);
 }
 #endif
 
diff --git a/mpas-model_amd/mpas_dycore/dycore.py b/mpas-model_amd/mpas_dycore/dycore.py
--- a/mpas-model_amd/mpas_dycore/dycore.py
+++ b/mpas-model_amd/mpas_dycore/dycore.py
@@ -444,7 +444,8 @@
 
     def folded_passes(self) -> tuple:
         m = int(self.lib.mpas_dyc_folded_passes(self.h))
-        return tuple(n for i, n in enumerate(("substep_avg", "rk1_edges", "recover_diag")) if m & (1 << i))
+        names = ("substep_avg", "rk1_edges", "recover_diag", "stage_avg_stores", "derived_coefs")
+        return tuple(n for i, n in enumerate(names) if m & (1 << i))
 
     def exchange_profile(self, dt: float, itimestep: int = 1) -> dict:
         self._check(self.lib.mpas_dyc_set_profile(self.h, 1), "set_profile")
```

Result: faster. 275.3 million cell-updates/s, median of 6 (+3.3%).
